# AwsGeek/thinvids

Hardware: AMD Instinct MI355X
Metric: encoded frames/sec (whole node) at fixed PSNR, 1080p & 4K HEVC, 1/2/4/8 MI355X (higher is better)
Workload: dtype uint8 video / int32 integer transforms (bit-exact HEVC)

## Files before the change

### csrc/core/capi.cpp

```cpp
#include <cstring>
#include <exception>
#include <memory>
#include <string>
#include <vector>

#include "tv/av1_enc.h"
#include "tv/container.h"
#include "tv/cpu_encoder.h"
#include "tv/hevc_codec.h"
#include "tv/me_model.h"
#include "tv/sdh.h"
#include "tv/synth.h"
#include "tv/synth_tile.h"
#include "tv/tb_frag.h"

using namespace tv;

namespace {
thread_local std::string g_err;
template <class F> int guard(F&& f) {
  try {
    f();
    return 0;
  } catch (const std::exception& e) {
    g_err = e.what();
    return -1;
  }
}
struct Bytes {
  std::vector<uint8_t> v;
};

struct TileOctave {
  int nx = 0;
  std::vector<uint8_t> lat;
  std::vector<uint16_t> top;
  std::vector<int> cy, sy;
  void build(int lp, uint32_t seed, const std::vector<int32_t>& px, const std::vector<int32_t>& py) {
    const SynthWin w = synth_win(lp, seed, px.front(), px.back(), py.front(), py.back());
    nx = (int)px.size();
    lat.resize((size_t)w.npx * w.npy);
    for (int r = 0; r < w.npy; ++r)
      for (int i = 0; i < w.npx; ++i) lat[(size_t)r * w.npx + i] = (uint8_t)synth_win_lattice(w, i, r);
    top.resize((size_t)w.npy * nx);
    for (int x = 0; x < nx; ++x) {
      int ci, sx;
      synth_axis(px[x], w.sh, w.cx0, ci, sx);
      for (int r = 0; r < w.npy; ++r)
        top[(size_t)r * nx + x] = (uint16_t)synth_top(lat[(size_t)r * w.npx + ci], lat[(size_t)r * w.npx + ci + 1], sx);
    }
    cy.resize(py.size());
    sy.resize(py.size());
    for (size_t y = 0; y < py.size(); ++y) synth_axis(py[y], w.sh, w.cy0, cy[y], sy[y]);
  }
  int at(int x, int y) const {
    const uint16_t* t = &top[(size_t)cy[y] * nx + x];
    return synth_rows(t[0], t[nx], sy[y]);
  }
};

void synth_tile_fill(const SynthFrameCtx& f, int c, int x0, int y0, int nx, int ny, int pw, uint8_t* P) {
  const int s = c ? 1 : 0, dw = c ? f.W / 2 : f.W, dh = c ? f.H / 2 : f.H;
  const bool tex = synth_textured(f.seed);
  std::vector<int32_t> px(nx), py(ny), qx(nx), qy(ny);
  for (int x = 0; x < nx; ++x) px[x] = synth_tile_pos(x0 + x, dw, s);
  for (int y = 0; y < ny; ++y) py[y] = synth_tile_pos(y0 + y, dh, s);
  std::vector<int> v((size_t)nx * ny);
  TileOctave oct[4];
  for (int x = 0; x < nx; ++x) qx[x] = px[x] + f.t * synth_pan_x(tex);
  for (int y = 0; y < ny; ++y) qy[y] = py[y] + f.t * synth_pan_y(tex);
  const int nb = synth_bg_octaves(c, tex);
  for (int i = 0; i < nb; ++i) oct[i].build(synth_bg_lp(c, i), synth_bg_seed(f.seed, c, i), qx, qy);
  for (int y = 0; y < ny; ++y)
    for (int x = 0; x < nx; ++x) {
      int n[4] = {0, 0, 0, 0};
      for (int i = 0; i < nb; ++i) n[i] = oct[i].at(x, y);
      v[(size_t)y * nx + x] = synth_bg_mix(c, tex, n);
    }
  for (int k = 0; k < kSynthObjects; ++k) {
    const SynthObject& o = f.obj[k];
    int32_t xlo, xhi, ylo, yhi;
    synth_obj_range(px.front(), px.back(), f.ox[k], o.w, xlo, xhi);
    synth_obj_range(py.front(), py.back(), f.oy[k], o.h, ylo, yhi);
    if (xlo > xhi || ylo > yhi) continue;
    for (int x = 0; x < nx; ++x) qx[x] = clip3(xlo, xhi, px[x] - f.ox[k]);
    for (int y = 0; y < ny; ++y) qy[y] = clip3(ylo, yhi, py[y] - f.oy[k]);
    const int no = synth_obj_octaves(c), base = synth_obj_base(f.seed, k, c);
    for (int i = 0; i < no; ++i) oct[i].build(synth_obj_lp(c, i), synth_obj_seed(o, c, i), qx, qy);
    for (int y = 0; y < ny; ++y)
      for (int x = 0; x < nx; ++x) {
        const int32_t rx16 = px[x] - f.ox[k], ry16 = py[y] - f.oy[k];
        if (rx16 != qx[x] || ry16 != qy[y] || synth_cover_col(o, rx16) > synth_cover_row(o, ry16)) continue;
        int n[2] = {0, 0};
        for (int i = 0; i < no; ++i) n[i] = oct[i].at(x, y);
        v[(size_t)y * nx + x] = synth_obj_mix(c, base, n);
      }
  }
  for (int y = 0; y < ny; ++y)
    for (int x = 0; x < nx; ++x) {
      int r = v[(size_t)y * nx + x];
      if (tex) r += synth_grain(f.seed, f.t, c, tv_min(x0 + x, dw - 1), tv_min(y0 + y, dh - 1));
      P[(size_t)(y0 + y) * pw + x0 + x] = (uint8_t)clip_pixel(r);
    }
}
}

extern "C" {

const char* tv_last_error() { return g_err.c_str(); }
int tv_core_version() { return 1; }

void* tv_bytes_new() { return new Bytes(); }
void tv_bytes_free(void* b) { delete static_cast<Bytes*>(b); }
size_t tv_bytes_size(void* b) { return static_cast<Bytes*>(b)->v.size(); }
const uint8_t* tv_bytes_data(void* b) { return static_cast<Bytes*>(b)->v.data(); }
void tv_bytes_clear(void* b) { static_cast<Bytes*>(b)->v.clear(); }

void tv_synth_frame(uint32_t seed, int t, int W, int H, uint8_t* y, uint8_t* u, uint8_t* v) {
  SynthFrameCtx ctx;
  synth_frame_ctx(seed, t, W, H, ctx);
  for (int c = 0; c < 3; ++c) {
    uint8_t* P = c == 0 ? y : (c == 1 ? u : v);
    const int w = c ? W / 2 : W, h = c ? H / 2 : H;
    for (int j = 0; j < h; ++j)
      for (int i = 0; i < w; ++i) P[(size_t)j * w + i] = (uint8_t)synth_sample_ctx(ctx, c, i, j);
  }
}

void tv_synth_frame_tiled(uint32_t seed, int t, int W, int H, int tile_w, int tile_h, uint8_t* y, uint8_t* u,
                          uint8_t* v) {
  SynthFrameCtx ctx;
  synth_frame_ctx(seed, t, W, H, ctx);
  const int cw = (W + kCtb - 1) / kCtb * kCtb, ch = (H + kCtb - 1) / kCtb * kCtb;
  for (int c = 0; c < 3; ++c) {
    uint8_t* P = c == 0 ? y : (c == 1 ? u : v);
    const int pw = c ? cw / 2 : cw, ph = c ? ch / 2 : ch;
    for (int y0 = 0; y0 < ph; y0 += tile_h)
      for (int x0 = 0; x0 < pw; x0 += tile_w)
        synth_tile_fill(ctx, c, x0, y0, tv_min(tile_w, pw - x0), tv_min(tile_h, ph - y0), pw, P);
  }
}

int tv_satd8x8(const int* d, int stride) { return satd8x8(d, stride); }

void* tv_cpu_encoder_new(int width, int height, int qp, int deblock, int range, int max_merge) {
  SeqConfig cfg;
  cfg.width = width;
  cfg.height = height;
  cfg.qp = qp;
  cfg.set_flags(deblock);
  cfg.max_merge_cand = max_merge;
  cfg.finalize();
  CpuEncoder* e = nullptr;
  guard([&] { e = new CpuEncoder(cfg, range); });
  return e;
}
void* tv_cpu_encoder_new_b(int width, int height, int qp, int deblock, int range, int max_merge, int mgop) {
  SeqConfig cfg;
  cfg.width = width;
  cfg.height = height;
  cfg.qp = qp;
  cfg.set_flags(deblock);
  cfg.max_merge_cand = max_merge;
  cfg.mgop = mgop;
  cfg.finalize();
  CpuEncoder* e = nullptr;
  guard([&] { e = new CpuEncoder(cfg, range); });
  return e;
}
int tv_cpu_encoder_begin_gop(void* e, int nframes, int* disp) {
  return guard([&] {
    auto* enc = static_cast<CpuEncoder*>(e);
    enc->begin_gop(nframes);
    for (size_t k = 0; k < enc->plan().pics.size(); ++k) disp[k] = enc->plan().pics[k].disp;
  });
}
int tv_gop_plan(int nframes, int mgop, int* disp, int* type, int* ref0, int* ref1, int* layer, int* info) {
  const GopPlan g = plan_gop(nframes, mgop);
  for (size_t k = 0; k < g.pics.size(); ++k) {
    disp[k] = g.pics[k].disp;
    type[k] = g.pics[k].type;
    ref0[k] = g.pics[k].ref[0];
    ref1[k] = g.pics[k].ref[1];
    layer[k] = g.pics[k].layer;
  }
  info[0] = g.dpb_size;
  info[1] = g.num_reorder;
  return (int)g.pics.size();
}
void* tv_cpu_encoder_new_crf(int width, int height, int qp, int deblock, int range, int max_merge, int crf) {
  SeqConfig cfg;
  cfg.width = width;
  cfg.height = height;
  cfg.qp = qp;
  cfg.set_flags(deblock);
  cfg.max_merge_cand = max_merge;
  cfg.crf = crf;
  cfg.finalize();
  CpuEncoder* e = nullptr;
  guard([&] { e = new CpuEncoder(cfg, range); });
  return e;
}
void tv_cpu_encoder_free(void* e) { delete static_cast<CpuEncoder*>(e); }
int tv_cpu_encoder_encode(void* e, const uint8_t* y, const uint8_t* u, const uint8_t* v, int sy,
                          int sc, int idr, int poc, void* out) {
  return guard([&] {
    const uint8_t* planes[3] = {y, u, v};
    const int strides[3] = {sy, sc, sc};
    static_cast<CpuEncoder*>(e)->encode_frame(planes, strides, idr != 0, poc, static_cast<Bytes*>(out)->v);
  });
}
int tv_cpu_encoder_encode_qp(void* e, const uint8_t* y, const uint8_t* u, const uint8_t* v, int sy, int sc, int idr,
                             int poc, int qp, void* out) {
  return guard([&] {
    const uint8_t* planes[3] = {y, u, v};
    const int strides[3] = {sy, sc, sc};
    static_cast<CpuEncoder*>(e)->encode_frame(planes, strides, idr != 0, poc, static_cast<Bytes*>(out)->v, qp);
  });
}
void tv_cpu_encoder_recon(void* e, uint8_t* y, uint8_t* u, uint8_t* v) {
  const Picture& p = static_cast<CpuEncoder*>(e)->recon();
  std::memcpy(y, p.y.data(), p.y.size());
  std::memcpy(u, p.u.data(), p.u.size());
  std::memcpy(v, p.v.data(), p.v.size());
}
void tv_cpu_encoder_decisions(void* e, uint8_t* cu_log2, uint8_t* intra, uint8_t* ipm, int16_t* mv,
                              uint8_t* cbf) {
  const FrameDecisions& d = static_cast<CpuEncoder*>(e)->dec;
  std::memcpy(cu_log2, d.cu_log2.data(), d.cu_log2.size());
  std::memcpy(intra, d.intra.data(), d.intra.size());
  std::memcpy(ipm, d.ipm.data(), d.ipm.size());
  std::memcpy(mv, d.mv.data(), d.mv.size() * 2);
  std::memcpy(cbf, d.cbf.data(), d.cbf.size());
}
void tv_cpu_encoder_levels(void* e, int16_t* cy, int16_t* cu, int16_t* cv) {
  const FrameDecisions& d = static_cast<CpuEncoder*>(e)->dec;
  std::memcpy(cy, d.coef_y.data(), d.coef_y.size() * 2);
  std::memcpy(cu, d.coef_u.data(), d.coef_u.size() * 2);
  std::memcpy(cv, d.coef_v.data(), d.coef_v.size() * 2);
}

int tv_reconstruct_frame(int width, int height, int qp, int deblock, const uint8_t* src_y,
                         const uint8_t* src_u, const uint8_t* src_v, const uint8_t* ref_y,
                         const uint8_t* ref_u, const uint8_t* ref_v, const uint8_t* cu_log2,
                         const uint8_t* intra, const uint8_t* ipm, const int16_t* mv,
                         uint8_t* cbf_out, int16_t* cy, int16_t* cu, int16_t* cv, uint8_t* rec_y,
                         uint8_t* rec_u, uint8_t* rec_v) {
  return guard([&] {
    SeqConfig cfg;
    cfg.width = width;
    cfg.height = height;
    cfg.qp = qp;
    cfg.deblock = (deblock & ~kFlagSignHiding) != 0;
    cfg.sign_hiding = (deblock & kFlagSignHiding) != 0;
    cfg.rqt = false;
    cfg.finalize();
    const int W = cfg.coded_w, H = cfg.coded_h;
    Picture src, ref, rec;
    src.alloc(W, H);
    rec.alloc(W, H);
    std::memcpy(src.y.data(), src_y, src.y.size());
    std::memcpy(src.u.data(), src_u, src.u.size());
    std::memcpy(src.v.data(), src_v, src.v.size());
    if (ref_y) {
      ref.alloc(W, H);
      std::memcpy(ref.y.data(), ref_y, ref.y.size());
      std::memcpy(ref.u.data(), ref_u, ref.u.size());
      std::memcpy(ref.v.data(), ref_v, ref.v.size());
    }
    FrameDecisions fd;
    fd.alloc(W, H);
    std::memcpy(fd.cu_log2.data(), cu_log2, fd.cu_log2.size());
    std::memcpy(fd.intra.data(), intra, fd.intra.size());
    std::memcpy(fd.ipm.data(), ipm, fd.ipm.size());
    std::memcpy(fd.mv.data(), mv, fd.mv.size() * 2);
    reconstruct_frame(cfg, src, ref_y ? &ref : nullptr, fd, rec);
    std::memcpy(cbf_out, fd.cbf.data(), fd.cbf.size());
    std::memcpy(cy, fd.coef_y.data(), fd.coef_y.size() * 2);
    std::memcpy(cu, fd.coef_u.data(), fd.coef_u.size() * 2);
    std::memcpy(cv, fd.coef_v.data(), fd.coef_v.size() * 2);
    std::memcpy(rec_y, rec.y.data(), rec.y.size());
    std::memcpy(rec_u, rec.u.data(), rec.u.size());
    std::memcpy(rec_v, rec.v.data(), rec.v.size());
  });
}

int tv_write_frame(int width, int height, int qp, int deblock, int max_merge, int idr, int poc,
                   const uint8_t* cu_log2, const uint8_t* intra, const uint8_t* ipm,
                   const int16_t* mv, const uint8_t* cbf, const int16_t* cy, const int16_t* cu,
                   const int16_t* cv, void* out) {
  return guard([&] {
    SeqConfig cfg;
    cfg.width = width;
    cfg.height = height;
    cfg.qp = qp;
    cfg.deblock = (deblock & ~kFlagSignHiding) != 0;
    cfg.sign_hiding = (deblock & kFlagSignHiding) != 0;
    cfg.max_merge_cand = max_merge;
    cfg.finalize();
    FrameData f;
    f.w8 = cfg.w8();
    f.h8 = cfg.h8();
    f.cu_log2 = cu_log2;
    f.intra = intra;
    f.ipm = ipm;
    f.mv = mv;
    f.cbf = cbf;
    f.coef[0] = cy;
    f.coef[1] = cu;
    f.coef[2] = cv;
    auto& o = static_cast<Bytes*>(out)->v;
    if (idr) write_parameter_sets(cfg, o);
    write_slice(cfg, f, poc, idr != 0, o);
  });
}

void* tv_decoder_new() { return new HevcDecoder(); }
void tv_decoder_free(void* d) { delete static_cast<HevcDecoder*>(d); }
int tv_decoder_decode(void* d, const uint8_t* data, size_t n) {
  return guard([&] { static_cast<HevcDecoder*>(d)->decode(data, n); });
}
int tv_decoder_decode_range(void* d, const uint8_t* data, size_t n, int first, int count) {
  return guard([&] { static_cast<HevcDecoder*>(d)->decode_range(data, n, first, count); });
}
void tv_hevc_scale_mv(int mvx, int mvy, int td, int tb, int* out) {
  const Mv m = scale_mv(Mv{mvx, mvy}, td, tb);
  out[0] = m.x;
  out[1] = m.y;
}
int tv_hevc_display_offsets(const uint8_t* data, size_t n, int* out, int cap) {
  int r = -1;
  guard([&] {
    const std::vector<int> off = display_offsets(data, n);
    for (int i = 0; i < (int)off.size() && i < cap; ++i) out[i] = off[i];
    r = (int)off.size();
  });
  return r;
}
int tv_hevc_probe(const uint8_t* data, size_t n, int* w, int* h, int* pictures, int* idrs) {
  return guard([&] {
    const StreamInfo s = probe_annexb(data, n);
    *w = s.width;
    *h = s.height;
    *pictures = s.pictures;
    *idrs = s.idrs;
  });
}
void tv_decoder_info(void* d, int* w, int* h, int* cw, int* ch, int* nframes) {
  auto* D = static_cast<HevcDecoder*>(d);
  *w = D->width;
  *h = D->height;
  *cw = D->coded_w;
  *ch = D->coded_h;
  *nframes = (int)D->pictures.size();
}
int tv_decoder_frame(void* d, int idx, int cropped, uint8_t* y, uint8_t* u, uint8_t* v) {
  return guard([&] {
    auto* D = static_cast<HevcDecoder*>(d);
    const Picture& p = D->pictures.at(idx).pic;
    const int w = cropped ? D->width : p.w, h = cropped ? D->height : p.h;
    for (int c = 0; c < 3; ++c) {
      uint8_t* dst = c == 0 ? y : (c == 1 ? u : v);
      const int cw = c ? w / 2 : w, chh = c ? h / 2 : h, sw = p.pw(c);
      for (int j = 0; j < chh; ++j) std::memcpy(dst + (size_t)j * cw, p.plane(c) + (size_t)j * sw, cw);
    }
  });
}

int tv_mux_mp4(const uint8_t* annexb, size_t n, int w, int h, int fps_num, int fps_den, void* out) {
  return guard([&] { static_cast<Bytes*>(out)->v = mux_mp4(annexb, n, w, h, fps_num, fps_den); });
}
int tv_mux_mp4_file(const uint8_t* const* segs, const size_t* sizes, int nseg, int w, int h, int fps_num, int fps_den,
                    const char* path, unsigned long long* out_size) {
  return guard([&] { *out_size = mux_mp4_file(segs, sizes, nseg, w, h, fps_num, fps_den, path); });
}
int tv_mux_file(const uint8_t* const* segs, const size_t* sizes, int nseg, int w, int h, int fps_num, int fps_den,
                const SideTrack* tracks, int ntracks, int container, const char* path, unsigned long long* out_size) {
  return guard([&] {
    *out_size = mux_file(segs, sizes, nseg, w, h, fps_num, fps_den, tracks, ntracks, container, path);
  });
}
size_t tv_side_track_size() { return sizeof(SideTrack); }

void tv_mv_rate(const int* dx, const int* dy, int n, int* est, int* idx) {
  for (int i = 0; i < n; ++i) {
    est[i] = mv_bits_est(dx[i], dy[i]);
    idx[i] = me_pen_index(dx[i], dy[i]);
  }
}
void tv_av1_mv_comp_bits(const int* d, int n, int* bits) {
  for (int i = 0; i < n; ++i) bits[i] = av1::mv_comp_bits(d[i]);
}
int tv_tb_frag_expand(int which, int* out) {
  static constexpr TbFragTables t = make_tb_frag();
  if (which < 0 || which >= 8) return 0;
  const int side = which < 2 ? 32 : 16;
  for (int n = 0; n < side; ++n)
    for (int k = 0; k < side; ++k)
      out[n * side + k] = int_of_f16_bits(which < 2 ? t.t32[which][n][k] : t.c16[(which - 2) >> 1][which & 1][n][k]);
  return side;
}
void tv_quant_levels(const int* coef, int n, int qp, int log2N, int* ref, int* fast) {
  const QuantParams q = quant_params(qp, log2N);
  for (int i = 0; i < n; ++i) {
    ref[i] = quant_level(coef[i], qp, log2N, false);
    fast[i] = quant_fast(coef[i], q);
  }
}
void tv_sdh_deltas(const int* coef, int n, int qp, int log2N, int intra, int* ref, int* fast) {
  const QuantParams q = quant_params(qp, log2N);
  for (int i = 0; i < n; ++i) {
    const int l = quant_level(coef[i], qp, log2N, intra != 0);
    ref[i] = sdh_delta(coef[i], l, qp, log2N);
    fast[i] = sdh_delta_fast(coef[i], l, q);
  }
}
int tv_demux_mp4(const uint8_t* mp4, size_t n, int* w, int* h, int* nframes, int* timescale,
                 int* delta, void* out) {
  return guard([&] { static_cast<Bytes*>(out)->v = demux_mp4(mp4, n, w, h, nframes, timescale, delta); });
}

}
```

### csrc/gpu/k_frame.hip

```cpp
#include <cstring>

#include "gpu_common.h"
#include "k_encode.h"
#include "tv/synth.h"
#include "tv/synth_tile.h"

namespace tv {
namespace gpu {

constexpr int kSynTW = kSynthTileW, kSynTH = kSynthTileH, kSynRows = kSynTH / 4;
static_assert(kSynTW == 256 && kSynTH % 4 == 0, "a wave of 4-sample items spans the tile; 4 waves share its rows");

struct SynthArgs {
  SynthObject obj[kSynthObjects];
  int32_t t[kMaxBatch];
  int32_t ox[kMaxBatch][kSynthObjects], oy[kMaxBatch][kSynthObjects];
};
static_assert(sizeof(SynthArgs) + sizeof(Geo) + sizeof(FrameSet) + 16 <= 4096, "kernel arguments are limited to 4 KB");

constexpr int kSynSpanX = (kSynTW - 1) * 16, kSynSpanY = (kSynTH - 1) * 16;
constexpr int syn_max(int a, int b) { return a > b ? a : b; }
constexpr int syn_pts(int lp, int s) { return synth_win_max(kSynSpanX << s, lp) * synth_win_max(kSynSpanY << s, lp); }
constexpr int syn_rows(int lp, int s) { return synth_win_max(kSynSpanY << s, lp); }
constexpr int syn_lat_size(bool tex) {
  return syn_max(syn_max(syn_pts(7, 0) + syn_pts(5, 0) + syn_pts(3, 0) + (tex ? syn_pts(1, 0) : 0), syn_pts(4, 0) + syn_pts(2, 0)),
                 syn_max(syn_pts(8, 1), syn_pts(5, 1)));
}
constexpr int syn_top_rows(bool tex) {
  return syn_max(syn_max(syn_rows(7, 0) + syn_rows(5, 0) + syn_rows(3, 0) + (tex ? syn_rows(1, 0) : 0), syn_rows(4, 0) + syn_rows(2, 0)),
                 syn_max(syn_rows(8, 1), syn_rows(5, 1)));
}

__device__ __forceinline__ void syn_lattice(const SynthWin& w, uint8_t* lat, int wave, int lane) {
  for (int r = wave; r < w.npy; r += 4)
    for (int i = lane; i < w.npx; i += 64) lat[r * w.npx + i] = (uint8_t)synth_win_lattice(w, i, r);
}
__device__ __forceinline__ void syn_top(const SynthWin& w, const uint8_t* lat, uint16_t* top, int col, int32_t p16) {
  int ci, sx;
  synth_axis(p16, w.sh, w.cx0, ci, sx);
  for (int r = 0; r < w.npy; ++r)
    top[r * kSynTW + col] = (uint16_t)synth_top(lat[r * w.npx + ci], lat[r * w.npx + ci + 1], sx);
}
__device__ __forceinline__ void syn_eval(const SynthWin& w, const uint16_t* top, int x, int32_t p16, int n[4]) {
  int cy, sy;
  synth_axis(p16, w.sh, w.cy0, cy, sy);
  const uint2 a = *reinterpret_cast<const uint2*>(top + cy * kSynTW + x);
  const uint2 b = *reinterpret_cast<const uint2*>(top + (cy + 1) * kSynTW + x);
  n[0] = synth_rows((int)(a.x & 0xffff), (int)(b.x & 0xffff), sy);
  n[1] = synth_rows((int)(a.x >> 16), (int)(b.x >> 16), sy);
  n[2] = synth_rows((int)(a.y & 0xffff), (int)(b.y & 0xffff), sy);
  n[3] = synth_rows((int)(a.y >> 16), (int)(b.y >> 16), sy);
}

template <bool kTex, bool kChroma>
__device__ __forceinline__ void syn_tile(uint16_t* top, uint8_t* lat, FrameSet src, const Geo& g, uint32_t seed,
                                         const SynthArgs& a, int c, int x0, int y0) {
  constexpr int kBg = kChroma ? 1 : (kTex ? 4 : 3), kOb = kChroma ? 1 : 2, s = kChroma ? 1 : 0;
  __builtin_assume(kChroma ? c != 0 : c == 0);
  const int b = blockIdx.y;
  const int pw = g.W >> s, ph = g.H >> s, dw = g.dw >> s, dh = g.dh >> s;
  const int t = a.t[b];
  const int tid = threadIdx.x, lane = tid & 63, wave = __builtin_amdgcn_readfirstlane(tid >> 6);
  const int32_t tx0 = synth_tile_pos(x0, dw, s), tx1 = synth_tile_pos(x0 + kSynTW - 1, dw, s);
  const int32_t ty0 = synth_tile_pos(y0, dh, s), ty1 = synth_tile_pos(y0 + kSynTH - 1, dh, s);
  const int32_t colp = synth_tile_pos(x0 + tid, dw, s);
  const int x = 4 * lane, yw = y0 + wave * kSynRows;
  int32_t sp[4];
#pragma unroll
  for (int j = 0; j < 4; ++j) sp[j] = synth_tile_pos(x0 + x + j, dw, s);

  SynthWin w[kBg];
  int lat0[kBg], row0[kBg];
  const int panx = t * synth_pan_x(kTex), pany = t * synth_pan_y(kTex);
  {
    int lo = 0, ro = 0;
#pragma unroll
    for (int i = 0; i < kBg; ++i) {
      w[i] = synth_win(synth_bg_lp(c, i), synth_bg_seed(seed, c, i), tx0 + panx, tx1 + panx, ty0 + pany, ty1 + pany);
      lat0[i] = lo;
      row0[i] = ro;
      syn_lattice(w[i], lat + lo, wave, lane);
      lo += w[i].npx * w[i].npy;
      ro += w[i].npy;
    }
  }
  __syncthreads();
#pragma unroll
  for (int i = 0; i < kBg; ++i) syn_top(w[i], lat + lat0[i], top + row0[i] * kSynTW, tid, colp + panx);
  __syncthreads();
  uint32_t word[kSynRows];
#pragma unroll
  for (int j = 0; j < kSynRows; ++j) {
    const int32_t py = synth_tile_pos(yw + j, dh, s) + pany;
    int n[4][4] = {};
#pragma unroll
    for (int i = 0; i < kBg; ++i) syn_eval(w[i], top + row0[i] * kSynTW, x, py, n[i]);
    word[j] = 0;
#pragma unroll
    for (int q = 0; q < 4; ++q) {
      const int m[4] = {n[0][q], n[1][q], n[2][q], n[3][q]};
      word[j] |= (uint32_t)synth_bg_mix(c, kTex, m) << (8 * q);
    }
  }

  for (int k = 0; k < kSynthObjects; ++k) {
    const SynthObject& o = a.obj[k];
    const int32_t ox = a.ox[b][k], oy = a.oy[b][k];
    int32_t xlo, xhi, ylo, yhi;
    synth_obj_range(tx0, tx1, ox, o.w, xlo, xhi);
    synth_obj_range(ty0, ty1, oy, o.h, ylo, yhi);
    if (xlo > xhi || ylo > yhi) continue;
    const int base = synth_obj_base(seed, k, c);
    SynthWin wo[kOb];
    int olat[kOb], orow[kOb];
    __syncthreads();
    {
      int lo = 0, ro = 0;
#pragma unroll
      for (int i = 0; i < kOb; ++i) {
        wo[i] = synth_win(synth_obj_lp(c, i), synth_obj_seed(o, c, i), xlo, xhi, ylo, yhi);
        olat[i] = lo;
        orow[i] = ro;
        syn_lattice(wo[i], lat + lo, wave, lane);
        lo += wo[i].npx * wo[i].npy;
        ro += wo[i].npy;
      }
    }
    __syncthreads();
#pragma unroll
    for (int i = 0; i < kOb; ++i) syn_top(wo[i], lat + olat[i], top + orow[i] * kSynTW, tid, clip3(xlo, xhi, colp - ox));
    __syncthreads();
    int64_t cover[4];
#pragma unroll
    for (int q = 0; q < 4; ++q) {
      const int32_t rx16 = sp[q] - ox;
      cover[q] = rx16 < xlo || rx16 > xhi ? INT64_MAX : synth_cover_col(o, rx16);
    }
#pragma unroll
    for (int j = 0; j < kSynRows; ++j) {
      const int32_t ry16 = synth_tile_pos(yw + j, dh, s) - oy;
      if (ry16 < ylo || ry16 > yhi) continue;
      const int64_t cover_row = synth_cover_row(o, ry16);
      int n[2][4] = {};
#pragma unroll
      for (int i = 0; i < kOb; ++i) syn_eval(wo[i], top + orow[i] * kSynTW, x, ry16, n[i]);
#pragma unroll
      for (int q = 0; q < 4; ++q) {
        if (cover[q] > cover_row) continue;
        const int m[2] = {n[0][q], n[1][q]};
        word[j] = (word[j] & ~(0xffu << (8 * q))) | (uint32_t)synth_obj_mix(c, base, m) << (8 * q);
      }
    }
  }

  if (x0 + x >= pw) return;
  uint8_t* P = src.plane(c, b, g);
#pragma unroll
  for (int j = 0; j < kSynRows; ++j) {
    const int y = yw + j;
    if (y >= ph) break;
    uint32_t out = word[j];
    if (kTex) {
      const int yc = tv_min(y, dh - 1);
      out = 0;
#pragma unroll
      for (int q = 0; q < 4; ++q) {
        const int v = (int)((word[j] >> (8 * q)) & 255) + synth_grain(seed, t, c, tv_min(x0 + x + q, dw - 1), yc);
        out |= (uint32_t)clip_pixel(v) << (8 * q);
      }
    }
    *reinterpret_cast<uint32_t*>(P + (long)y * pw + x0 + x) = out;
  }
}

template <bool kTex>
__global__ void __launch_bounds__(256) k_synth(FrameSet src, Geo g, uint32_t seed, SynthArgs a) {
  __shared__ __attribute__((aligned(8))) uint16_t top[syn_top_rows(kTex) * kSynTW];
  __shared__ uint8_t lat[syn_lat_size(kTex)];
  const int nlx = (g.W + kSynTW - 1) / kSynTW, ncx = (g.W / 2 + kSynTW - 1) / kSynTW;
  const int nl = nlx * ((g.H + kSynTH - 1) / kSynTH), nc = ncx * ((g.H / 2 + kSynTH - 1) / kSynTH);
  int id = blockIdx.x, c = 0;
  if (id >= nl) {
    c = id >= nl + nc ? 2 : 1;
    id -= nl + (c - 1) * nc;
  }
  const int ntx = c ? ncx : nlx, ty = id / ntx, x0 = (id - ty * ntx) * kSynTW, y0 = ty * kSynTH;
  if (c)
    syn_tile<kTex, true>(top, lat, src, g, seed, a, c, x0, y0);
  else
    syn_tile<kTex, false>(top, lat, src, g, seed, a, 0, x0, y0);
}

__global__ void __launch_bounds__(256) k_sse(FrameSet a, FrameSet r, Geo g, unsigned long long* sse) {
  const int c = blockIdx.y, b = blockIdx.z;
  const int pw = c ? g.W / 2 : g.W;
  const int dw = c ? g.dw / 2 : g.dw, dh = c ? g.dh / 2 : g.dh;
  const uint8_t* A = a.plane(c, b, g);
  const uint8_t* R = r.plane(c, b, g);
  const int wq = (dw + 3) >> 2;
  unsigned s = 0;
  for (int i = blockIdx.x * blockDim.x + threadIdx.x; i < wq * dh; i += gridDim.x * blockDim.x) {
    const int y = i / wq, x = (i - y * wq) * 4;
    const uint32_t va = *reinterpret_cast<const uint32_t*>(A + (long)y * pw + x);
    const uint32_t vr = *reinterpret_cast<const uint32_t*>(R + (long)y * pw + x);
#pragma unroll
    for (int k = 0; k < 4; ++k) {
      const int d = (int)((va >> (8 * k)) & 255) - (int)((vr >> (8 * k)) & 255);
      s += (x + k < dw) ? (unsigned)(d * d) : 0u;
    }
  }
  unsigned long long t = s;
  for (int o = 32; o > 0; o >>= 1) t += __shfl_xor(t, o, 64);
  __shared__ unsigned long long part[4];
  if ((threadIdx.x & 63) == 0) part[threadIdx.x >> 6] = t;
  __syncthreads();
  if (threadIdx.x == 0) atomicAdd(sse + b * 3 + c, part[0] + part[1] + part[2] + part[3]);
}

typedef short tv_short2 __attribute__((ext_vector_type(2)));

__device__ constexpr uint32_t pack_taps4(int f, int k0) {
  return (uint32_t)(uint8_t)kLumaFilter[f][k0] | (uint32_t)(uint8_t)kLumaFilter[f][k0 + 1] << 8 |
         (uint32_t)(uint8_t)kLumaFilter[f][k0 + 2] << 16 | (uint32_t)(uint8_t)kLumaFilter[f][k0 + 3] << 24;
}
__device__ constexpr uint32_t pack_taps2(int f, int k0) {
  return (uint32_t)(uint16_t)kLumaFilter[f][k0] | (uint32_t)(uint16_t)kLumaFilter[f][k0 + 1] << 16;
}
__device__ __forceinline__ int dot4(uint32_t a, uint32_t b, int c) {
  return __builtin_amdgcn_sdot4((int)a, (int)b, c, false);
}
__device__ __forceinline__ int dot2(uint32_t a, uint32_t b, int c) {
  return __builtin_amdgcn_sdot2(__builtin_bit_cast(tv_short2, a), __builtin_bit_cast(tv_short2, b), c, false);
}
__device__ __forceinline__ uint32_t pack4_pixels(int v0, int v1, int v2, int v3) {
  return (uint32_t)clip_pixel(v0) | (uint32_t)clip_pixel(v1) << 8 | (uint32_t)clip_pixel(v2) << 16 |
         (uint32_t)clip_pixel(v3) << 24;
}

constexpr int kPhW = 10;
__global__ void __launch_bounds__(256) k_phase_planes(FrameSet ref, uint8_t* phase, Geo g) {
  const int tid = threadIdx.x;
  const int L = xcd_remap(blockIdx.x + gridDim.x * (blockIdx.y + gridDim.y * blockIdx.z),
                          gridDim.x * gridDim.y * gridDim.z);
  const int tpf = gridDim.x * gridDim.y, b = L / tpf, tyi = (L - b * tpf) / gridDim.x;
  const int tx0 = (L - b * tpf - tyi * gridDim.x) * 32 - 8, ty0 = tyi * 32 - 8;
  const uint8_t* R = ref.plane(0, b, g);
  __shared__ uint32_t raw[39][kPhW];
  __shared__ __align__(16) int16_t hf[3][39][32];
  for (int i = tid; i < 39 * kPhW; i += 256) {
    const int rr = i / kPhW, w = i - rr * kPhW;
    const uint8_t* row = R + (long)clip3(0, g.H - 1, ty0 - 3 + rr) * g.W;
    const int x = tx0 - 4 + 4 * w;
    uint32_t v;
    if (x >= 0 && x + 3 < g.W) {
      v = *reinterpret_cast<const uint32_t*>(row + x);
    } else {
      v = 0;
#pragma unroll
      for (int k = 0; k < 4; ++k) v |= (uint32_t)row[clip3(0, g.W - 1, x + k)] << (8 * k);
    }
    raw[rr][w] = v ^ 0x80808080u;
  }
  __syncthreads();
  for (int i = tid; i < 39 * 8; i += 256) {
    const int rr = i >> 3, c4 = i & 7;
    const uint32_t w0 = raw[rr][c4], w1 = raw[rr][c4 + 1], w2 = raw[rr][c4 + 2];
    int out[3][4];
#pragma unroll
    for (int j = 0; j < 4; ++j) {
      const uint32_t lo = j == 3 ? w1 : __builtin_amdgcn_alignbyte(w1, w0, j + 1);
      const uint32_t hi = j == 3 ? w2 : __builtin_amdgcn_alignbyte(w2, w1, j + 1);
#pragma unroll
      for (int f = 1; f < 4; ++f) out[f - 1][j] = dot4(lo, pack_taps4(f, 0), dot4(hi, pack_taps4(f, 4), 8192));
    }
#pragma unroll
    for (int f = 0; f < 3; ++f) {
      uint2 v;
      v.x = (uint32_t)(uint16_t)out[f][0] | (uint32_t)out[f][1] << 16;
      v.y = (uint32_t)(uint16_t)out[f][2] | (uint32_t)out[f][3] << 16;
      *reinterpret_cast<uint2*>(&hf[f][rr][4 * c4]) = v;
    }
  }
  __syncthreads();
  const int r = tid >> 3, c0 = (tid & 7) * 4;
  const int X = tx0 + c0, Y = ty0 + r;
  if (X + 8 >= g.pw16 || Y >= g.H + 8) return;
  uint8_t* base = phase + (long)b * 16 * g.psz + (long)(Y + 8) * g.pw16 + (X + 8);
  auto store = [&](int plane, uint32_t w) { *reinterpret_cast<uint32_t*>(base + (long)plane * g.psz) = w; };
  {
    uint32_t R8[8];
#pragma unroll
    for (int k = 0; k < 8; ++k) R8[k] = raw[r + k][(c0 >> 2) + 1];
    store(0, R8[3] ^ 0x80808080u);
    uint32_t C[2][4];
#pragma unroll
    for (int h = 0; h < 2; ++h) {
      const uint32_t* q = R8 + 4 * h;
      const uint32_t t01l = __builtin_amdgcn_perm(q[1], q[0], 0x05010400u);
      const uint32_t t01h = __builtin_amdgcn_perm(q[1], q[0], 0x07030602u);
      const uint32_t t23l = __builtin_amdgcn_perm(q[3], q[2], 0x05010400u);
      const uint32_t t23h = __builtin_amdgcn_perm(q[3], q[2], 0x07030602u);
      C[h][0] = __builtin_amdgcn_perm(t23l, t01l, 0x05040100u);
      C[h][1] = __builtin_amdgcn_perm(t23l, t01l, 0x07060302u);
      C[h][2] = __builtin_amdgcn_perm(t23h, t01h, 0x05040100u);
      C[h][3] = __builtin_amdgcn_perm(t23h, t01h, 0x07060302u);
    }
#pragma unroll
    for (int fy = 1; fy < 4; ++fy) {
      int v[4];
#pragma unroll
      for (int j = 0; j < 4; ++j)
        v[j] = dot4(C[0][j], pack_taps4(fy, 0), dot4(C[1][j], pack_taps4(fy, 4), 8192 + 32)) >> 6;
      store(4 * fy, pack4_pixels(v[0], v[1], v[2], v[3]));
    }
  }
#pragma unroll
  for (int fx = 1; fx < 4; ++fx) {
    uint2 H8[8];
#pragma unroll
    for (int k = 0; k < 8; ++k) H8[k] = *reinterpret_cast<const uint2*>(&hf[fx - 1][r + k][c0]);
    {
      const int h0 = (int16_t)(H8[3].x & 0xffff), h1 = (int16_t)(H8[3].x >> 16);
      const int h2 = (int16_t)(H8[3].y & 0xffff), h3 = (int16_t)(H8[3].y >> 16);
      store(fx, pack4_pixels((h0 + 32) >> 6, (h1 + 32) >> 6, (h2 + 32) >> 6, (h3 + 32) >> 6));
    }
    uint32_t P[4][4];
#pragma unroll
    for (int m = 0; m < 4; ++m) {
      P[m][0] = __builtin_amdgcn_perm(H8[2 * m + 1].x, H8[2 * m].x, 0x05040100u);
      P[m][1] = __builtin_amdgcn_perm(H8[2 * m + 1].x, H8[2 * m].x, 0x07060302u);
      P[m][2] = __builtin_amdgcn_perm(H8[2 * m + 1].y, H8[2 * m].y, 0x05040100u);
      P[m][3] = __builtin_amdgcn_perm(H8[2 * m + 1].y, H8[2 * m].y, 0x07060302u);
    }
#pragma unroll
    for (int fy = 1; fy < 4; ++fy) {
      int v[4];
#pragma unroll
      for (int j = 0; j < 4; ++j) {
        int a = dot2(P[0][j], pack_taps2(fy, 0), 0);
        a = dot2(P[1][j], pack_taps2(fy, 2), a);
        a = dot2(P[2][j], pack_taps2(fy, 4), a);
        a = dot2(P[3][j], pack_taps2(fy, 6), a);
        v[j] = ((a >> 6) + 32) >> 6;
      }
      store(fx + 4 * fy, pack4_pixels(v[0], v[1], v[2], v[3]));
    }
  }
}

__global__ void __launch_bounds__(256) __attribute__((amdgpu_waves_per_eu(8, 8))) k_deblock(FrameSet rec, DecisionSet dec, Geo g, int horizontal) {
  const int b = blockIdx.y;
  const int qp = dec.qp[b];
  const long ub = b * g.usz;
  const uint8_t* cl = dec.cu_log2 + ub;
  const uint8_t* in = dec.intra + ub;
  const uint8_t* cb = dec.cbf + ub;
  const int16_t* mv = dec.mv + 2 * ub;
  const uint8_t* dir = dec.dir ? dec.dir + ub : nullptr;
  const int16_t* mv1 = dec.mv1 ? dec.mv1 + 2 * ub : nullptr;
  const uint8_t* tu = dec.tu ? dec.tu + ub : nullptr;
  uint8_t* Y = rec.plane(0, b, g);
  uint8_t* U = rec.plane(1, b, g);
  uint8_t* V = rec.plane(2, b, g);
  const int W = g.W, H = g.H, Wc = W / 2;
  const int qpc = chroma_qp(qp, 0);
  const int nl = horizontal ? (H / 8 - 1) * (W / 4) : (W / 8 - 1) * (H / 4);
  const int nc = horizontal ? (H / 16 - 1) * (Wc / 4) : (W / 16 - 1) * (H / 8);
  auto ld = [](const uint8_t* p) { return *reinterpret_cast<const uint32_t*>(p); };
  auto st = [](uint8_t* p, uint32_t v) { *reinterpret_cast<uint32_t*>(p) = v; };
  for (int i = blockIdx.x * blockDim.x + threadIdx.x; i < nl + nc; i += gridDim.x * blockDim.x) {
    if (i < nl) {
      if (!horizontal) {
        const int x = 8 * (1 + i % (W / 8 - 1)), y = 4 * (i / (W / 8 - 1));
        const int bs = deblock_edge_bs(cl, in, cb, mv, g.w8, x - 1, y, x, y, dir, mv1, tu);
        if (bs) {
          uint32_t v[4][2];
#pragma unroll
          for (int k = 0; k < 4; ++k) {
            v[k][0] = ld(Y + (long)(y + k) * W + x - 4);
            v[k][1] = ld(Y + (long)(y + k) * W + x);
          }
          deblock_luma_edge4(reinterpret_cast<uint8_t*>(&v[0][1]), 1, 8, bs, qp);
#pragma unroll
          for (int k = 0; k < 4; ++k) {
            st(Y + (long)(y + k) * W + x - 4, v[k][0]);
            st(Y + (long)(y + k) * W + x, v[k][1]);
          }
        }
      } else {
        const int y = 8 * (1 + i % (H / 8 - 1)), x = 4 * (i / (H / 8 - 1));
        const int bs = deblock_edge_bs(cl, in, cb, mv, g.w8, x, y - 1, x, y, dir, mv1, tu);
        if (bs) {
          uint32_t v[8];
#pragma unroll
          for (int r = 0; r < 8; ++r) v[r] = ld(Y + (long)(y - 4 + r) * W + x);
          deblock_luma_edge4(reinterpret_cast<uint8_t*>(&v[4]), 4, 1, bs, qp);
#pragma unroll
          for (int r = 1; r < 7; ++r) st(Y + (long)(y - 4 + r) * W + x, v[r]);
        }
      }
    } else {
      const int j = i - nl;
      if (!horizontal) {
        const int xc = 8 * (1 + j % (W / 16 - 1)), yc = 4 * (j / (W / 16 - 1));
        const int bs = deblock_edge_bs(cl, in, cb, mv, g.w8, 2 * xc - 1, 2 * yc, 2 * xc, 2 * yc, dir, mv1, tu);
        if (bs == 2) {
#pragma unroll
          for (int pl = 0; pl < 2; ++pl) {
            uint8_t* P = pl ? V : U;
            uint32_t v[4][2];
#pragma unroll
            for (int k = 0; k < 4; ++k) {
              v[k][0] = ld(P + (long)(yc + k) * Wc + xc - 4);
              v[k][1] = ld(P + (long)(yc + k) * Wc + xc);
            }
            deblock_chroma_edge(reinterpret_cast<uint8_t*>(&v[0][1]), 1, 8, 4, qpc);
#pragma unroll
            for (int k = 0; k < 4; ++k) {
              st(P + (long)(yc + k) * Wc + xc - 4, v[k][0]);
              st(P + (long)(yc + k) * Wc + xc, v[k][1]);
            }
          }
        }
      } else {
        const int yc = 8 * (1 + j % (H / 16 - 1)), xc = 4 * (j / (H / 16 - 1));
        const int bs = deblock_edge_bs(cl, in, cb, mv, g.w8, 2 * xc, 2 * yc - 1, 2 * xc, 2 * yc, dir, mv1, tu);
        if (bs == 2) {
#pragma unroll
          for (int pl = 0; pl < 2; ++pl) {
            uint8_t* P = pl ? V : U;
            uint32_t v[4];
#pragma unroll
            for (int r = 0; r < 4; ++r) v[r] = ld(P + (long)(yc - 2 + r) * Wc + xc);
            deblock_chroma_edge(reinterpret_cast<uint8_t*>(&v[2]), 4, 1, 4, qpc);
            st(P + (long)(yc - 1) * Wc + xc, v[1]);
            st(P + (long)yc * Wc + xc, v[2]);
          }
        }
      }
    }
  }
}

void launch_synth(FrameSet src, const Geo& g, uint32_t seed, const FrameIdx& fi, int B, hipStream_t s) {
  SynthArgs a;
  std::memset(&a, 0, sizeof a);
  SynthFrameCtx f;
  for (int b = 0; b < B; ++b) {
    synth_frame_ctx(seed, fi.t[b], g.dw, g.dh, f);
    a.t[b] = f.t;
    std::memcpy(a.ox[b], f.ox, sizeof f.ox);
    std::memcpy(a.oy[b], f.oy, sizeof f.oy);
  }
  if (B > 0) std::memcpy(a.obj, f.obj, sizeof f.obj);
  auto tiles = [](int w, int h) { return ((w + kSynTW - 1) / kSynTW) * ((h + kSynTH - 1) / kSynTH); };
  dim3 grid((unsigned)(tiles(g.W, g.H) + 2 * tiles(g.W / 2, g.H / 2)), (unsigned)B);
  if (synth_textured(seed))
    k_synth<true><<<grid, 256, 0, s>>>(src, g, seed, a);
  else
    k_synth<false><<<grid, 256, 0, s>>>(src, g, seed, a);
}
__global__ void __launch_bounds__(256) k_gather_frames(const uint8_t* frames, long seg_stride, FrameSet src, Geo g,
                                                       int B) {
  const long f16 = (g.ysz + 2 * g.csz) / 16, y16 = g.ysz / 16, c16 = g.csz / 16;
  for (long i = (long)blockIdx.x * 256 + threadIdx.x; i < B * f16; i += (long)gridDim.x * 256) {
    const int b = (int)(i / f16);
    const long r = i - b * f16;
    const uint4 v = reinterpret_cast<const uint4*>(frames + b * seg_stride)[r];
    uint4* d = r < y16 ? reinterpret_cast<uint4*>(src.y + b * g.ysz) + r
               : r < y16 + c16 ? reinterpret_cast<uint4*>(src.u + b * g.csz) + (r - y16)
                               : reinterpret_cast<uint4*>(src.v + b * g.csz) + (r - y16 - c16);
    *d = v;
  }
}
void launch_gather_frames(const uint8_t* frames, long seg_stride, FrameSet src, const Geo& g, int B, hipStream_t s) {
  const long n = B * (g.ysz + 2 * g.csz) / 16;
  k_gather_frames<<<(unsigned)tv_min(4096L, (n + 255) / 256), 256, 0, s>>>(frames, seg_stride, src, g, B);
}
struct QpArgs {
  int8_t q[64];
};
__global__ void __launch_bounds__(64) k_set_qp(int8_t* dst, QpArgs a, int n) {
  if ((int)threadIdx.x < n) dst[threadIdx.x] = a.q[threadIdx.x];
}
void launch_set_qp(int8_t* dst, const int8_t* host, int n, hipStream_t s) {
  for (int o = 0; o < n; o += 64) {
    QpArgs a;
    const int m = n - o < 64 ? n - o : 64;
    std::memcpy(a.q, host + o, (size_t)m);
    k_set_qp<<<1, 64, 0, s>>>(dst + o, a, m);
  }
}

void launch_sse(FrameSet a, FrameSet r, const Geo& g, unsigned long long* sse, int B, hipStream_t s) {
  dim3 grid((unsigned)tv_min(256, (int)((g.ysz / 4 + 4095) / 4096)), 3, B);
  k_sse<<<grid, 256, 0, s>>>(a, r, g, sse);
}
void launch_phase_planes(FrameSet ref, uint8_t* phase, const Geo& g, int B, hipStream_t s) {
  dim3 grid((g.W + 16 + 31) / 32, (g.H + 16 + 31) / 32, B);
  k_phase_planes<<<grid, 256, 0, s>>>(ref, phase, g);
}
constexpr int kSaoT = 34;
constexpr int kSaoTc = 18;
constexpr int kSaoP = kSaoT + 2, kSaoPc = kSaoTc + 2;
constexpr int kSaoTile = kSaoT * kSaoP + 2 * kSaoTc * kSaoPc;
constexpr int kSaoStage = (kSaoTile + 255) / 256;
__device__ __forceinline__ int sao_tix(int c, int row, int col) {
  return c == 0 ? row * kSaoP + col + 1 : kSaoT * kSaoP + (c - 1) * kSaoTc * kSaoPc + row * kSaoPc + col + 1;
}
typedef short sao_s2 __attribute__((ext_vector_type(2)));
__device__ __forceinline__ sao_s2 sao_pair(uint32_t w) { return __builtin_bit_cast(sao_s2, w); }
typedef unsigned short sao_u2 __attribute__((ext_vector_type(2)));
__device__ __forceinline__ sao_s2 sao_sign2(sao_s2 d) {
  const sao_s2 z = {0, 0};
  const sao_u2 f = {15, 15};
  return (d >> 15) | __builtin_bit_cast(sao_s2, __builtin_bit_cast(sao_u2, z - d) >> f);
}
__device__ __forceinline__ sao_s2 sao_relu2(sao_s2 e) { return e & ~(e >> 15); }
__device__ __forceinline__ sao_s2 sao_pkmax(sao_s2 a, sao_s2 b) {
  uint32_t r;
  asm("v_pk_max_i16 %0, %1, %2" : "=v"(r) : "v"(__builtin_bit_cast(uint32_t, a)), "v"(__builtin_bit_cast(uint32_t, b)));
  return sao_pair(r);
}
__device__ __forceinline__ sao_s2 sao_pkmin(sao_s2 a, sao_s2 b) {
  uint32_t r;
  asm("v_pk_min_i16 %0, %1, %2" : "=v"(r) : "v"(__builtin_bit_cast(uint32_t, a)), "v"(__builtin_bit_cast(uint32_t, b)));
  return sao_pair(r);
}

__device__ __forceinline__ void sao_tile_pos(int i, int& c, int& j) {
  c = i < kSaoT * kSaoT ? 0 : (i < kSaoT * kSaoT + kSaoTc * kSaoTc ? 1 : 2);
  j = c == 0 ? i : i - kSaoT * kSaoT - (c - 1) * kSaoTc * kSaoTc;
}

__global__ void __launch_bounds__(256) k_sao_decide(FrameSet src, FrameSet deb, FrameSet out, uint32_t* sao, Geo g,
                                                    const int8_t* qp, const RcTables* rc,
                                                    unsigned long long* sse) {
  const int tid = threadIdx.x, lane = tid & 63;
  int ctu, b;
  xcd_ctb(ctu, b);
  const long long lam16 = rc->sao_lam16[qp[b]];
  const int cx = ctu % g.wc, cy = ctu / g.wc;
  __shared__ SaoStats st[3];
  __shared__ __align__(16) int16_t tile[kSaoTile];
  __shared__ int bpos[3];
  __shared__ int bh[3][32][16];
  for (int i = tid; i < 3 * (int)(sizeof(SaoStats) / 4); i += 256) reinterpret_cast<int*>(st)[i] = 0;
  if (kSaoBandOffsets)
    for (int i = tid; i < 3 * 32 * 16; i += 256) (&bh[0][0][0])[i] = 0;
  {
    uint32_t* tile32 = reinterpret_cast<uint32_t*>(tile);
    uint32_t v[3];
    int at[3], dw[3], nd[3];
    bool act[3], in[3];
#pragma unroll
    for (int k = 0; k < 3; ++k) {
      int c, row, d;
      if (k < 2) {
        const int i = tid + 256 * k;
        c = 0;
        row = i / 10;
        d = i - 10 * row;
        act[k] = i < 34 * 10;
      } else {
        const int pl = tid >= 108 ? 1 : 0, j = tid - 108 * pl;
        c = 1 + pl;
        row = j / 6;
        d = j - 6 * row;
        act[k] = tid < 2 * 108;
      }
      const int n = c ? 16 : 32, w = c ? g.W / 2 : g.W, h = c ? g.H / 2 : g.H;
      const int x = cx * n - 4 + 4 * d, y = cy * n - 1 + row;
      in[k] = act[k] && x >= 0 && x < w && y >= 0 && y < h;
      v[k] = in[k] ? *reinterpret_cast<const uint32_t*>(deb.plane(c, b, g) + (long)y * w + x) : 0u;
      at[k] = (sao_tix(c, row, -1) >> 1) + 2 * d - 1;
      dw[k] = d;
      nd[k] = c ? 6 : 10;
    }
#pragma unroll
    for (int k = 0; k < 3; ++k) {
      if (!act[k]) continue;
      const uint32_t lo = in[k] ? __builtin_amdgcn_perm(0u, v[k], 0x0c010c00u) : 0xFFFFFFFFu;
      const uint32_t hi = in[k] ? __builtin_amdgcn_perm(0u, v[k], 0x0c030c02u) : 0xFFFFFFFFu;
      if (dw[k] >= 1) tile32[at[k]] = lo;
      if (dw[k] < nd[k] - 1) tile32[at[k] + 1] = hi;
    }
  }
  const int wave = __builtin_amdgcn_readfirstlane(tid >> 6);
  const int c = wave < 2 ? 0 : wave - 1;
  const int n = c ? 16 : 32, w = c ? g.W / 2 : g.W;
  const int nsh = c ? 4 : 5;
  const int iters = c ? 4 : 8;
  const uint8_t* S = src.plane(c, b, g) + (long)(cy * n) * w + cx * n;
  static_assert(!kSaoBandOffsets, "the packed statistics carry no band histogram");
  const bool interior = cx > 0 && cy > 0 && cx < g.wc - 1 && cy < g.hc - 1;
  const int piters = c ? 2 : 4;
  int sv[8] = {};
  uint32_t sp[4] = {};
  if (interior) {
#pragma unroll
    for (int k = 0; k < 4; ++k) {
      const int pidx = lane + 64 * k;
      const int ly = (c == 0 ? wave * 16 : 0) + (pidx >> (nsh - 1)), lx = 2 * (pidx & ((n >> 1) - 1));
      sp[k] = k < piters ? *reinterpret_cast<const uint16_t*>(S + ly * w + lx) : 0u;
    }
  } else {
#pragma unroll
    for (int k = 0; k < 8; ++k) {
      const int i = (c == 0 ? wave * 512 : 0) + lane + 64 * k;
      sv[k] = k < iters ? S[(i >> nsh) * w + (i & (n - 1))] : 0;
    }
  }
  __syncthreads();
  int eo[4][4];
  if (interior) {
    const uint32_t* tile32 = reinterpret_cast<const uint32_t*>(tile);
    sao_s2 acc[4][4];
#pragma unroll
    for (int d = 0; d < 4; ++d)
#pragma unroll
      for (int q = 0; q < 4; ++q) acc[d][q] = sao_s2{0, 0};
    const sao_s2 zero = {0, 0}, one = {1, 1}, mone = {-1, -1}, sixteen = {16, 16};
#pragma unroll
    for (int k = 0; k < 4; ++k) {
      if (k >= piters) break;
      const int pidx = lane + 64 * k;
      const int ly = (c == 0 ? wave * 16 : 0) + (pidx >> (nsh - 1)), lx = 2 * (pidx & ((n >> 1) - 1));
      uint32_t Pv[3], Cv[3], Nv[3];
#pragma unroll
      for (int r = 0; r < 3; ++r) {
        const int i0 = sao_tix(c, ly + r, lx + 1) >> 1;
        Pv[r] = tile32[i0 - 1];
        Cv[r] = tile32[i0];
        Nv[r] = tile32[i0 + 1];
      }
      sao_s2 L[3], R[3], Cc[3];
#pragma unroll
      for (int r = 0; r < 3; ++r) {
        L[r] = sao_pair(__builtin_amdgcn_alignbyte(Cv[r], Pv[r], 2));
        R[r] = sao_pair(__builtin_amdgcn_alignbyte(Nv[r], Cv[r], 2));
        Cc[r] = sao_pair(Cv[r]);
      }
      const sao_s2 v = Cc[1];
      const uint32_t o = sp[k];
      const sao_s2 orig = {(short)(o & 255), (short)(o >> 8)};
      const sao_s2 w = (orig - v) * sixteen + one;
      const sao_s2 A[4] = {L[1], Cc[0], L[0], R[0]}, Bn[4] = {R[1], Cc[2], R[2], L[2]};
#pragma unroll
      for (int d = 0; d < 4; ++d) {
        const sao_s2 e = sao_pkmin(sao_pkmax(v - A[d], mone), one) + sao_pkmin(sao_pkmax(v - Bn[d], mone), one);
        const sao_s2 pos = sao_pkmax(e, zero), neg = sao_pkmax(zero - e, zero);
        const sao_s2 is[4] = {neg >> one, neg & one, pos & one, pos >> one};
#pragma unroll
        for (int q = 0; q < 4; ++q) acc[d][q] += w * is[q];
      }
    }
#pragma unroll
    for (int d = 0; d < 4; ++d)
#pragma unroll
      for (int q = 0; q < 4; ++q) {
        const int F = __builtin_amdgcn_sdot2(acc[d][q], one, 0, false), C = F & 15;
        eo[d][q] = (F - C) * 128 + C;
      }
  } else {
    unsigned long long eo64[4] = {0, 0, 0, 0};
#pragma unroll
    for (int k = 0; k < 8; ++k) {
      if (k >= iters) break;
      const int i = (c == 0 ? wave * 512 : 0) + lane + 64 * k;
      const int lx = i & (n - 1), ly = i >> nsh;
      const int v = tile[sao_tix(c, ly + 1, lx + 1)];
      const int d16 = (sv[k] - v) * 16 + 1;
      const unsigned long long p64 = (unsigned long long)(long long)d16;
#pragma unroll
      for (int d = 0; d < 4; ++d) {
        int dx, dy;
        sao_eo_dir(d, dx, dy);
        const int a = tile[sao_tix(c, ly + 1 + dy, lx + 1 + dx)], bb = tile[sao_tix(c, ly + 1 - dy, lx + 1 - dx)];
        const int e = tv_min(tv_max(v - a, -1), 1) + tv_min(tv_max(v - bb, -1), 1);
        const int f = e + 2 - (e > 0);
        eo64[d] += (a >= 0 && bb >= 0 && e != 0) ? p64 << (16 * f) : 0ull;
      }
      if (kSaoBandOffsets) atomicAdd(&bh[c][v >> 3][lane & 15], (sv[k] - v) * 2048 + 1);
    }
#pragma unroll
    for (int d = 0; d < 4; ++d) {
      unsigned long long acc = eo64[d];
#pragma unroll
      for (int q = 0; q < 4; ++q) {
        const int fv = (int)(int16_t)(acc & 0xffffu);
        acc = (acc - (unsigned long long)(long long)fv) >> 16;
        const int cnt = fv & 15;
        eo[d][q] = ((fv - cnt) >> 4) * 2048 + cnt;
      }
    }
  }
  {
    int t[16];
#pragma unroll
    for (int k = 0; k < 16; ++k) t[k] = eo[k >> 2][k & 3];
#pragma unroll
    for (int j = 0; j < 8; ++j) {
      const auto r = __builtin_amdgcn_permlane32_swap((unsigned)t[j], (unsigned)t[j + 8], false, false);
      t[j] = (int)(r[0] + r[1]);
    }
#pragma unroll
    for (int j = 0; j < 4; ++j) {
      const auto r = __builtin_amdgcn_permlane16_swap((unsigned)t[j], (unsigned)t[j + 4], false, false);
      t[j] = (int)(r[0] + r[1]);
    }
    const int m8 = -((lane >> 3) & 1), m4 = -((lane >> 2) & 1);
#pragma unroll
    for (int j = 0; j < 2; ++j) {
      const int x = (t[j] ^ t[j + 2]) & m8;
      t[j] = (t[j] ^ x) + dpp::mov<dpp::kRowRor8>(t[j + 2] ^ x);
    }
    {
      const int x = (t[0] ^ t[1]) & m4;
      t[0] = (t[0] ^ x) + __shfl_xor(t[1] ^ x, 4, 64);
    }
    int tot = t[0];
    tot += dpp::mov<dpp::kQuadXor1>(tot);
    tot += dpp::mov<dpp::kQuadXor2>(tot);
    const int k = lane >> 2;
    if ((lane & 3) == 0 && (tot & 2047)) {
      atomicAdd(&st[c].eo_n[k >> 2][(k & 3) + 1], tot & 2047);
      atomicAdd(&st[c].eo_s[k >> 2][(k & 3) + 1], (tot - (tot & 2047)) / 2048);
    }
  }
  __shared__ SaoTables tab;
  __shared__ uint32_t prm[3];
  __syncthreads();
  if (kSaoBandOffsets && tid < 96) {
    const int cc = tid >> 5, band = tid & 31;
    int tot = 0;
#pragma unroll
    for (int k = 0; k < 16; ++k) tot += bh[cc][band][k];
    st[cc].bo_n[band] = tot & 2047;
    st[cc].bo_s[band] = (tot - (tot & 2047)) / 2048;
  }
  __syncthreads();
  if (tid < kSaoItems && (kSaoBandOffsets || tid % 48 < 16)) sao_item(st, lam16, tid, tab);
  __syncthreads();
  if (kSaoBandOffsets && tid < 96) sao_window(tid, tab);
  __syncthreads();
  if (!kSaoBandOffsets) {
    if (tid < 3) bpos[tid] = 0;
  } else if (wave < 3) {
    long long j = lane < 32 ? tab.win_j[wave][lane] : LLONG_MAX;
    int p = lane < 32 ? lane : 64;
#pragma unroll
    for (int o = 32; o >= 1; o >>= 1) {
      const long long j2 = __shfl_xor(j, o);
      const int p2 = __shfl_xor(p, o);
      if (j2 < j || (j2 == j && p2 < p)) {
        j = j2;
        p = p2;
      }
    }
    if (lane == 0) bpos[wave] = p;
  }
  __syncthreads();
  if (tid == 0) {
    sao_finish_pos(tab, lam16, bpos, prm);
    uint32_t* o = sao + 3 * ((long)b * g.wc * g.hc + ctu);
    o[0] = prm[0];
    o[1] = prm[1];
    o[2] = prm[2];
  }
  __syncthreads();
  static_assert(!kSaoBandOffsets, "the SAO filter has no band-offset path");
  unsigned e2[3] = {0, 0, 0};
  const uint32_t* tile32 = reinterpret_cast<const uint32_t*>(tile);
  for (int i = tid; i < 256 + 128; i += 256) {
    const int cc = i < 256 ? 0 : (i < 320 ? 1 : 2);
    const int j = cc == 0 ? i : i - 256 - (cc - 1) * 64;
    const int nd = cc ? 4 : 8, nn = cc ? 16 : 32, ww = cc ? g.W / 2 : g.W;
    const int ly = j >> (cc ? 2 : 3), lx0 = 4 * (j & (nd - 1));
    const uint32_t p = prm[cc];
    const long at = (long)(cy * nn + ly) * ww + cx * nn + lx0;
    const int dwc = cc ? g.dw / 2 : g.dw, dhc = cc ? g.dh / 2 : g.dh;
    const bool want_sse = sse && cy * nn + ly < dhc;
    const uint32_t sw = want_sse ? *reinterpret_cast<const uint32_t*>(src.plane(cc, b, g) + at) : 0u;
    uint32_t word = 0;
    const int i0 = sao_tix(cc, ly + 1, lx0 + 1) >> 1;
    const uint32_t C0 = tile32[i0], C1 = tile32[i0 + 1];
    if (sao_type(p) == 2) {
      int dx, dy;
      sao_eo_dir(sao_class(p), dx, dy);
      const int pd = (cc ? kSaoPc : kSaoP) >> 1;
      const int ra = i0 + dy * pd, rb = i0 - dy * pd;
      const uint32_t Wa[4] = {tile32[ra - 1], tile32[ra], tile32[ra + 1], tile32[ra + 2]};
      const uint32_t Wb[4] = {tile32[rb - 1], tile32[rb], tile32[rb + 1], tile32[rb + 2]};
      auto shifted = [](const uint32_t* W, int k, int s) -> uint32_t {
        return s == 0 ? W[k + 1] : s < 0 ? __builtin_amdgcn_alignbyte(W[k + 1], W[k], 2)
                                         : __builtin_amdgcn_alignbyte(W[k + 2], W[k + 1], 2);
      };
      const uint32_t t0 = ((p >> 7) & 15) | ((p >> 11) & 15) << 8 | 8u << 16 | ((p >> 15) & 15) << 24;
      const uint32_t t1 = (p >> 19) & 15;
      const sao_s2 two = {2, 2}, eight = {8, 8};
      const sao_u2 u8s = {8, 8};
      uint32_t r2[2];
#pragma unroll
      for (int k = 0; k < 2; ++k) {
        const sao_s2 v = sao_pair(k ? C1 : C0);
        const sao_s2 A = sao_pair(shifted(Wa, k, dx)), B = sao_pair(shifted(Wb, k, -dx));
        const sao_s2 inv = (A | B) >> 15;
        const sao_s2 e = (sao_sign2(v - A) + sao_sign2(v - B)) & ~inv;
        const uint32_t sel = __builtin_bit_cast(uint32_t, e + two) | 0x0c000c00u;
        const sao_s2 off = sao_pair(__builtin_amdgcn_perm(t1, t0, sel));
        const sao_s2 r = sao_relu2(v + off - eight);
        r2[k] = __builtin_bit_cast(uint32_t, r | (sao_s2{0, 0} - __builtin_bit_cast(sao_s2, __builtin_bit_cast(sao_u2, r) >> u8s)));
      }
      word = __builtin_amdgcn_perm(r2[1], r2[0], 0x06040200u);
    } else {
      word = __builtin_amdgcn_perm(C1, C0, 0x06040200u);
    }
    *reinterpret_cast<uint32_t*>(out.plane(cc, b, g) + at) = word;
    if (want_sse) {
      if (cx * nn + lx0 + 4 <= dwc) {
#pragma unroll
        for (int h = 0; h < 2; ++h) {
          const uint32_t sel = h ? 0x0c030c02u : 0x0c010c00u;
          const sao_s2 d = sao_pair(__builtin_amdgcn_perm(0u, sw, sel)) - sao_pair(__builtin_amdgcn_perm(0u, word, sel));
          const sao_u2 dd = __builtin_bit_cast(sao_u2, d * d);
          e2[cc] = __builtin_amdgcn_udot2(dd, sao_u2{1, 1}, e2[cc], false);
        }
      } else {
#pragma unroll
        for (int q = 0; q < 4; ++q) {
          const int d = (int)((sw >> (8 * q)) & 255) - (int)((word >> (8 * q)) & 255);
          e2[cc] += cx * nn + lx0 + q < dwc ? (unsigned)(d * d) : 0u;
        }
      }
    }
  }
  if (sse) {
    __shared__ unsigned long long esum[3];
    if (tid < 3) esum[tid] = 0;
    __syncthreads();
#pragma unroll
    for (int c2 = 0; c2 < 3; ++c2) {
      const int t = wave_sum((int)e2[c2]);
      if (lane == 0 && t) atomicAdd(&esum[c2], (unsigned long long)(unsigned)t);
    }
    __syncthreads();
    if (tid < 3 && esum[tid]) atomicAdd(sse + b * 3 + tid, esum[tid]);
  }
}

void launch_sao(FrameSet src, FrameSet deb, FrameSet out, uint32_t* sao, const int8_t* qp, const RcTables* rc,
                const Geo& g, int B, hipStream_t s, unsigned long long* sse) {
  k_sao_decide<<<dim3(g.wc * g.hc, B), 256, 0, s>>>(src, deb, out, sao, g, qp, rc, sse);
}

void launch_deblock(FrameSet rec, DecisionSet dec, const Geo& g, int B, hipStream_t s) {
  dim3 grid((unsigned)tv_min(1024, (int)(g.ysz / 32 / 256 + 1)), B);
  k_deblock<<<grid, 256, 0, s>>>(rec, dec, g, 0);
  k_deblock<<<grid, 256, 0, s>>>(rec, dec, g, 1);
}

}
}
```

### csrc/gpu/k_stage.hip

```cpp
#include <hip/hip_runtime.h>

#include <string>

#include "gpu_common.h"
#include "k_encode.h"

namespace tv {
namespace gpu {

__global__ void __launch_bounds__(256) k_pad_plane(const uint8_t* __restrict__ src, int sw, int sh, int sstride, long sfs,
                                                   uint8_t* __restrict__ dst, int pw, int ph, int dstride, long dfs) {
  const int f = blockIdx.z, y = blockIdx.y;
  const int x0 = (blockIdx.x * 256 + threadIdx.x) * 4;
  if (x0 >= pw) return;
  const uint8_t* S = src + f * sfs + (long)tv_min(y, sh - 1) * sstride;
  uint8_t* D = dst + f * dfs + (long)y * dstride;
#pragma unroll
  for (int k = 0; k < 4; ++k)
    if (x0 + k < pw) D[x0 + k] = S[tv_min(x0 + k, sw - 1)];
}

template <typename T>
__global__ void __launch_bounds__(256) k_thumbs8(const T* __restrict__ y, int tw, int stride, long fs, float* out,
                                                 float scale) {
  const int x = blockIdx.x * 256 + threadIdx.x, r = blockIdx.y, f = blockIdx.z;
  if (x >= tw) return;
  const T* p = y + (long)f * fs + (long)(8 * r) * stride + 8 * x;
  unsigned s = 0;
#pragma unroll
  for (int j = 0; j < 8; ++j)
#pragma unroll
    for (int i = 0; i < 8; ++i) s += p[(long)j * stride + i];
  out[((long)f * gridDim.y + r) * tw + x] = (float)s * scale / 64.0f;
}
}
}

namespace {
thread_local std::string g_stage_err;
int stage_status() {
  const hipError_t e = hipGetLastError();
  if (e == hipSuccess) return 0;
  g_stage_err = hipGetErrorString(e);
  return -1;
}
}

extern "C" {
const char* tv_stage_last_error() { return g_stage_err.c_str(); }

int tv_thumbs8_batch(const void* y, int bits, int w, int h, int stride, long fs, int n, float* out, void* stream) {
  const int tw = w / 8, th = h / 8;
  if (tw <= 0 || th <= 0 || th > 65535 || n <= 0 || n > 65535 || stride < w) {
    g_stage_err = "tv_thumbs8_batch: bad geometry";
    return -1;
  }
  const dim3 grid((unsigned)((tw + 255) / 256), (unsigned)th, (unsigned)n);
  hipStream_t st = static_cast<hipStream_t>(stream);
  if (bits > 8)
    tv::gpu::k_thumbs8<uint16_t><<<grid, 256, 0, st>>>(static_cast<const uint16_t*>(y), tw, stride, fs, out, 0.25f);
  else
    tv::gpu::k_thumbs8<uint8_t><<<grid, 256, 0, st>>>(static_cast<const uint8_t*>(y), tw, stride, fs, out, 1.0f);
  return stage_status();
}

int tv_pad_batch(const uint8_t* src, int sw, int sh, int sstride, long sfs, uint8_t* dst, int pw, int ph, int dstride,
                 long dfs, int n, void* stream) {
  if (sw <= 0 || sh <= 0 || pw < sw || ph < sh || dstride < pw || sstride < sw || n <= 0 || n > 65535 ||
      ph > 65535) {
    g_stage_err = "tv_pad_batch: bad geometry";
    return -1;
  }
  const dim3 grid((unsigned)((pw / 4 + 255) / 256 + 1), (unsigned)ph, (unsigned)n);
  tv::gpu::k_pad_plane<<<grid, 256, 0, static_cast<hipStream_t>(stream)>>>(src, sw, sh, sstride, sfs, dst, pw, ph,
                                                                          dstride, dfs);
  return stage_status();
}

int tv_synth_batch(uint8_t* dst, int w, int h, int n, const int* t, uint32_t seed, void* stream) {
  if (w < 2 || h < 2 || (w & 1) || (h & 1) || n <= 0) {
    g_stage_err = "tv_synth_batch: bad geometry";
    return -1;
  }
  const tv::gpu::Geo g = tv::gpu::make_geo(w, h);
  for (int b0 = 0; b0 < n; b0 += tv::gpu::kMaxBatch) {
    const int B = tv::tv_min(tv::gpu::kMaxBatch, n - b0);
    tv::gpu::FrameSet fs{dst + b0 * g.ysz, dst + n * g.ysz + b0 * g.csz, dst + n * g.ysz + n * g.csz + b0 * g.csz};
    tv::gpu::FrameIdx fi{};
    for (int b = 0; b < B; ++b) fi.t[b] = t[b0 + b];
    tv::gpu::launch_synth(fs, g, seed, fi, B, static_cast<hipStream_t>(stream));
  }
  return stage_status();
}
}
```

### thinvids_amd/_abi.py

```python
import ctypes as C

i, l, ll, sz, ull, f32 = C.c_int, C.c_long, C.c_longlong, C.c_size_t, C.c_ulonglong, C.c_float
i32, i64, u32, vp, cstr = C.c_int32, C.c_int64, C.c_uint32, C.c_void_p, C.c_char_p
u8p, i8p, i16p, i32p, u32p = (C.POINTER(t) for t in (C.c_uint8, C.c_int8, C.c_int16, C.c_int32, C.c_uint32))
i64p, u64p, lp, llp, ullp, szp = (C.POINTER(t) for t in (C.c_int64, C.c_uint64, l, ll, ull, sz))
f64p, vpp = C.POINTER(C.c_double), C.POINTER(vp)


class SideTrack(C.Structure):
    _fields_ = [("kind", i32), ("codec", i32), ("timescale", i32), ("channels", i32), ("sample_rate", i32),
                ("bits", i32), ("is_default", i32), ("reserved", i32), ("lang", C.c_char * 4), ("mkv_codec_id", cstr),
                ("priv", vp), ("priv_size", C.c_uint64), ("path", cstr), ("data", vp), ("nsamples", i64),
                ("offsets", vp), ("sizes", vp), ("pts", vp), ("durs", vp)]


CORE = {
    "tv_core_build_hash": (cstr, []),
    "tv_last_error": (cstr, []),
    "tv_core_version": (i, []),
    "tv_bytes_new": (vp, []),
    "tv_bytes_free": (None, [vp]),
    "tv_bytes_size": (sz, [vp]),
    "tv_bytes_data": (vp, [vp]),
    "tv_bytes_clear": (None, [vp]),
    "tv_synth_frame": (None, [u32, i, i, i, u8p, u8p, u8p]),
    "tv_synth_frame_tiled": (None, [u32, i, i, i, i, i, u8p, u8p, u8p]),
    "tv_satd8x8": (i, [i32p, i]),
    "tv_cpu_encoder_new": (vp, [i] * 6),
    "tv_cpu_encoder_new_b": (vp, [i] * 7),
    "tv_cpu_encoder_new_crf": (vp, [i] * 7),
    "tv_cpu_encoder_free": (None, [vp]),
    "tv_cpu_encoder_begin_gop": (i, [vp, i, i32p]),
    "tv_gop_plan": (i, [i, i] + [i32p] * 6),
    "tv_cpu_encoder_encode": (i, [vp, u8p, u8p, u8p, i, i, i, i, vp]),
    "tv_cpu_encoder_encode_qp": (i, [vp, u8p, u8p, u8p, i, i, i, i, i, vp]),
    "tv_cpu_encoder_recon": (None, [vp, u8p, u8p, u8p]),
    "tv_cpu_encoder_decisions": (None, [vp, u8p, u8p, u8p, i16p, u8p]),
    "tv_cpu_encoder_levels": (None, [vp, i16p, i16p, i16p]),
    "tv_reconstruct_frame": (i, [i] * 4 + [u8p] * 9 + [i16p, u8p, i16p, i16p, i16p, u8p, u8p, u8p]),
    "tv_write_frame": (i, [i] * 7 + [u8p, u8p, u8p, i16p, u8p, i16p, i16p, i16p, vp]),
    "tv_mv_rate": (None, [i32p, i32p, i, i32p, i32p]),
    "tv_av1_mv_comp_bits": (None, [i32p, i, i32p]),
    "tv_tb_frag_expand": (i, [i, i32p]),
    "tv_quant_levels": (None, [i32p, i, i, i, i32p, i32p]),
    "tv_sdh_deltas": (None, [i32p, i, i, i, i, i32p, i32p]),
    "tv_hevc_spec_table": (i, [cstr, i32p, i]),
    "tv_decoder_new": (vp, []),
    "tv_decoder_free": (None, [vp]),
    "tv_decoder_decode": (i, [vp, u8p, sz]),
    "tv_decoder_decode_range": (i, [vp, u8p, sz, i, i]),
    "tv_decoder_info": (None, [vp] + [i32p] * 5),
    "tv_decoder_frame": (i, [vp, i, i, u8p, u8p, u8p]),
    "tv_hevc_scale_mv": (None, [i, i, i, i, i32p]),
    "tv_hevc_display_offsets": (i, [u8p, sz, i32p, i]),
    "tv_hevc_probe": (i, [u8p, sz] + [i32p] * 4),
    "tv_mux_mp4": (i, [u8p, sz, i, i, i, i, vp]),
    "tv_mux_mp4_file": (i, [vpp, szp, i, i, i, i, i, cstr, ullp]),
    "tv_mux_file": (i, [vpp, szp, i, i, i, i, i, C.POINTER(SideTrack), i, i, cstr, ullp]),
    "tv_side_track_size": (sz, []),
    "tv_demux_mp4": (i, [u8p, sz] + [i32p] * 5 + [vp]),
    "tv_mp4s_open": (vp, [cstr, i, i, i, i, ull]),
    "tv_mp4s_append": (i, [vp, u8p, sz]),
    "tv_mp4s_close": (i, [vp, ullp]),
    "tv_mp4s_abort": (None, [vp]),
    "tv_mp4s_last_error": (cstr, []),
    "tv_io_last_error": (cstr, []),
    "tv_pread_parallel": (ll, [cstr, ll, ll, vp, i]),
    "tv_readahead": (i, [cstr, ll, ll]),
    "tv_av1c_last_error": (cstr, []),
    "tv_av1c_qlookup": (i, [i, i]),
    "tv_av1c_model_constants": (i, [i64p]),
    "tv_av1c_model_q": (None, [i, i64p]),
    "tv_av1c_golden_encode": (i, [i, i, i, u8p, i, i32p, i, vp, i64p, u8p, u32p, u32p, i16p, i16p, i16p, i32p, i8p,
                                  i32p, u8p]),
    "tv_av1c_ib_accept": (i, [u8p, i, i, u8p]),
    "tv_av1c_cfl_decide": (i, [u8p, u8p, u8p, i, i, i, i, i32p]),
    "tv_av1c_decode": (i, [u8p, sz, i, u8p, i32p, i32p]),
    "tv_av1c_probe": (i, [u8p, sz, i32p, i32p]),
    "tv_av1c_state_new": (vp, []),
    "tv_av1c_state_free": (None, [vp]),
    "tv_av1c_write_tu": (i, [vp, i, i, i32p, u32p, u32p, i16p, i16p, i16p, i8p, i32p, i, i, vp]),
    "tv_av1_last_error": (cstr, []),
    "tv_av1_cdef_find_dirs": (None, [u8p, i, i, u8p, i32p]),
    "tv_av1_cdef_search": (None, [u8p, u8p, i, i, i, u8p, i32p, i, i, u64p]),
    "tv_av1_cdef_apply": (None, [u8p, i, i, i, u8p, i32p, i, i, i8p, u8p]),
    "tv_av1_wiener_apply": (None, [u8p, i, i, i32p, u8p]),
    "tv_av1_wiener_stats": (None, [u8p, u8p, i, i, i, i32p, i64p]),
    "tv_av1_sgr_apply": (None, [u8p, i, i, i32p, u8p]),
    "tv_av1_sgr_stats": (None, [u8p, u8p, i, i, i, i64p]),
    "tv_av1_sgr_filter_planes": (None, [u8p, i, i, i, i32p, i32p]),
    "tv_av1_deblock": (i, [u8p, i, i, i, u32p, i, u8p]),
    "tv_av1_rc_roundtrip": (i, [i32p, i32p, i32p, i, i, i, vp, i32p]),
    "tv_av1_txfm_ref": (i, [i16p, i16p, i, i, i, i, i]),
    "tv_av1_txfm_basis": (i, [i, i, i32p]),
    "tv_mpeg2_last_error": (cstr, []),
    "tv_mpeg2_encode": (i, [i32p, i, i, u8p, vp, i64p, i32p, u8p]),
    "tv_mpeg2_probe": (i, [u8p, sz, i32p]),
    "tv_mpeg2_raps": (i, [u8p, sz, i64p, i64p, i32p, i32p, i]),
    "tv_mpeg2_decode": (i, [u8p, sz, i64, i64, i32, i32, i32, u8p, i32p, i64p]),
    "tv_mpeg2_table": (i, [i, i32p, i32p, i32p, i]),
    "tv_mpeg2_stat_name": (cstr, [i]),
    "tv_mpeg2_num_stats": (i, []),
}

GPU = {
    "tv_gpu_build_hash": (cstr, []),
    "tv_gpu_last_error": (cstr, []),
    "tv_gpu_device_count": (i, []),
    "tv_engine_new_b": (vp, [i] * 7 + [u32, i, i, i, i, i]),
    "tv_engine_free": (None, [vp]),
    "tv_engine_encode_synth": (i, [vp, i32p, i, i, vp]),
    "tv_engine_encode_host": (i, [vp, u8p, i, i, vp]),
    "tv_engine_encode_device": (i, [vp, vp, i, i, vp]),
    "tv_engine_segment_size": (sz, [vp, i]),
    "tv_engine_segment_copy": (None, [vp, i, u8p]),
    "tv_engine_sse": (None, [vp, i, f64p]),
    "tv_engine_timing": (None, [vp] + [f64p] * 4),
    "tv_engine_entropy_stats": (None, [vp, i32p, llp, i32p]),
    "tv_engine_entropy_host_pictures": (ll, [vp]),
    "tv_engine_entropy_lane_pictures": (ll, [vp, i]),
    "tv_engine_estimate": (i, [i] * 6 + [ullp, ullp]),
    "tv_engine_footprint": (None, [vp, ullp, ullp]),
    "tv_engine_last_recon": (i, [vp, i, u8p, u8p, u8p]),
    "tv_ingest_last_error": (cstr, []),
    "tv_ingest_h2d": (i, [cstr, ll, ll, vp, vp, ll, i, vp, f64p]),
    "tv_stage_last_error": (cstr, []),
    "tv_thumbs8_batch": (i, [vp, i, i, i, i, l, i, vp, vp]),
    "tv_pad_batch": (i, [vp, i, i, i, l, vp, i, i, i, l, i, vp]),
    "tv_synth_batch": (i, [vp, i, i, i, i32p, u32, vp]),
    "tv_ops_last_error": (cstr, []),
    "tv_resize_plane": (i, [vp, i, i, i, vp, i, i, i, vp, vp, i, vp, vp, i, vp, vp]),
    "tv_resize_batch": (i, [vp, i, i, i, l, vp, i, i, i, l, i, i, i, vp, vp, i, vp, vp, i, vp, i, i, i, vp]),
    "tv_rgb_to_i420": (i, [vp, i, i, i, vp, vp, vp, i, vp]),
    "tv_p010_to_i420": (i, [vp, vp, i, i, vp, vp, vp, vp]),
    "tv_tonemap_pq": (i, [vp, vp, i, i, vp, vp, vp, f32, f32, vp]),
    "tv_tonemap_pq_batch": (i, [vp, vp, i, i, i, vp, f32, f32, vp]),
    "tv_synth_p010": (i, [vp, vp, i, i, i, i, u32, vp]),
    "tv_overlay_mask": (i, [vp, i, i, i, vp, i, i, i, i, vp]),
    "tv_bwdif_segment": (i, [vp, vp, l, i, i, lp, i32p, i32p, i, vp]),
    "tv_bwdif_plane": (i, [vp, vp, vp, vp, i, i, i, vp]),
    "tv_ssim_plane": (i, [vp, vp, i, i, i, i, vp, vp]),
    "tv_av1_gpu_last_error": (cstr, []),
    "tv_gpu_cdef_dirs": (i, [vp, i, i, i, vp, vp, vp]),
    "tv_gpu_cdef_search": (i, [vp, vp, i, i, i, i, vp, vp, i, i, i, vp, vp, ull, i]),
    "tv_gpu_cdef_apply": (i, [vp, i, i, i, i, vp, vp, i, i, i, vp, vp, vp]),
    "tv_gpu_sgr_select": (i, [vp, vp, vp, i, i, i, i, vp, vp, vp, vp]),
    "tv_gpu_wiener_apply": (i, [vp, i, i, i, vp, vp, vp]),
    "tv_gpu_wiener_stats": (i, [vp, vp, i, i, i, i, vp, vp, vp]),
    "tv_gpu_sgr_stats": (i, [vp, vp, i, i, i, i, vp, vp]),
    "tv_gpu_sgr_apply": (i, [vp, i, i, i, vp, vp, vp]),
    "tv_gpu_av1_deblock_step": (i, [vp, vp, i, i, i, i, vp, i, i, vp]),
    "tv_av1_txfm_last_error": (cstr, []),
    "tv_gpu_av1_txfm": (i, [vp, vp, i, i, i, vp, vp, vp]),
    "tv_av1e_last_error": (cstr, []),
    "tv_av1e_inter": (i, [vp] * 18 + [i, i, i, vp, vp]),
    "tv_av1e_iblocks": (i, [vp] * 16 + [i, i, i, vp, i, vp]),
    "tv_av1e_intra": (i, [vp] * 11 + [i, i, i, vp, i, vp]),
    "tv_av1e_cdef_skip": (i, [vp, vp, i, i, i, vp]),
    "tv_av1e_merge": (i, [vp, vp, i, i, i, vp]),
    "tv_av1e_tb_len": (i, [vp, vp, l, i, i, i, i, vp, vp]),
    "tv_av1e_tb_pack": (i, [vp, vp, vp, l, i, i, i, i, vp, vp]),
    "tv_av1e_lfinfo": (i, [vp, i, i, i, vp, vp, vp, vp, vp]),
    "tv_av1e_unit_sse": (i, [vp, vp, i, i, i, i, i, vp, vp]),
    "tv_av1e_cdef_choose": (i, [vp, vp, vp, vp, i, i, i, vp, vp, vp, vp, vp]),
}
```

### thinvids_amd/models/hevc.py

```python
from __future__ import annotations

import ctypes as C
import threading
from dataclasses import dataclass

import numpy as np

from .._native import Bytes, check, core_lib, ok, ptr

Frame = tuple


def coded_size(width: int, height: int, ctb: int = 32) -> tuple[int, int]:
    return (width + ctb - 1) // ctb * ctb, (height + ctb - 1) // ctb * ctb


def synth_frame(seed: int, t: int, width: int, height: int) -> Frame:
    y = np.empty((height, width), np.uint8)
    u = np.empty((height // 2, width // 2), np.uint8)
    v = np.empty_like(u)
    core_lib().tv_synth_frame(seed & 0xFFFFFFFF, t, width, height, ptr(y), ptr(u), ptr(v))
    return y, u, v


def psnr(a: np.ndarray, b: np.ndarray) -> float:
    mse = np.mean((a.astype(np.float64) - b.astype(np.float64)) ** 2)
    return float("inf") if mse == 0 else 10.0 * np.log10(255.0 ** 2 / mse)


def psnr_yuv(ref: Frame, dec: Frame) -> dict:
    py, pu, pv = (psnr(r, d) for r, d in zip(ref, dec))
    return {"y": py, "u": pu, "v": pv, "yuv": (6 * py + pu + pv) / 8}


FLAG_DEBLOCK = 1
FLAG_SAO = 2
FLAG_WPP = 4
FLAG_NO_RQT = 8
FLAG_NO_PINTRA = 16
FLAG_HOST_ENTROPY = 32
FLAG_CASCADE = 64
FLAG_NO_RDOQ = 128
FLAG_SUBPEL_SATD = 256
FLAG_SIGN_HIDING = 512


def codec_flags(deblock: bool = True, sao: bool = False, wpp: bool = True, rqt: bool = True, pintra: bool = True,
                cascade: bool = False, rdoq: bool = True, subpel_satd: bool = False, sign_hiding: bool = False) -> int:
    on = {FLAG_DEBLOCK: deblock, FLAG_SAO: sao, FLAG_WPP: wpp, FLAG_NO_RQT: not rqt, FLAG_NO_PINTRA: not pintra,
          FLAG_CASCADE: cascade, FLAG_NO_RDOQ: not rdoq, FLAG_SUBPEL_SATD: subpel_satd, FLAG_SIGN_HIDING: sign_hiding}
    return sum(bit for bit, v in on.items() if v)


IPPP_CASCADE_IDR = -5
IPPP_CASCADE_P = (1, 0, 1, -1, 1, 0, 1, -3)


def ippp_cascade_qps(qp: int, nframes: int) -> list[int]:
    return [max(0, min(51, qp + (IPPP_CASCADE_IDR if i == 0 else IPPP_CASCADE_P[(i - 1) % 8]))) for i in range(nframes)]


class CpuEncoder:

    def __init__(self, width: int, height: int, qp: int = 27, deblock: bool = True,
                 search_range: int = 64, max_merge: int = 5, sao: bool = False, crf: int = 0, wpp: bool = True,
                 bframes: int = 1, rqt: bool = True, pintra: bool = True, cascade: bool = True, rdoq: bool = True,
                 subpel_satd: bool = False, sign_hiding: bool = False):
        if width % 2 or height % 2:
            raise ValueError("width/height must be even")
        self.lib = core_lib()
        self.width, self.height, self.qp = width, height, qp
        self.cw, self.ch = coded_size(width, height)
        self.bframes = int(bframes)
        flags = codec_flags(deblock, sao, wpp, rqt, pintra, cascade, rdoq, subpel_satd, sign_hiding)
        if self.bframes > 1:
            if crf:
                raise ValueError("CRF with B frames is not supported by the golden encoder")
            self.h = self.lib.tv_cpu_encoder_new_b(width, height, qp, flags, search_range, max_merge, self.bframes)
        elif crf:
            self.h = self.lib.tv_cpu_encoder_new_crf(width, height, qp, flags, search_range, max_merge, int(crf))
        else:
            self.h = self.lib.tv_cpu_encoder_new(width, height, qp, flags, search_range, max_merge)
        if not self.h:
            raise ValueError(self.lib.tv_last_error().decode())
        self.out = Bytes()

    def __del__(self):
        if getattr(self, "h", None):
            self.lib.tv_cpu_encoder_free(self.h)
            self.h = None

    def begin_gop(self, nframes: int) -> list[int]:
        disp = (C.c_int * nframes)()
        check(self.lib.tv_cpu_encoder_begin_gop(self.h, nframes, disp))
        return list(disp)

    def encode(self, frame: Frame, idr: bool, poc: int, qp: int | None = None) -> bytes:
        y, u, v = (np.ascontiguousarray(p) for p in frame)
        self.out.clear()
        if qp is None:
            check(self.lib.tv_cpu_encoder_encode(self.h, ptr(y), ptr(u), ptr(v), y.shape[1], u.shape[1],
                                                 int(idr), poc, self.out.h))
        else:
            check(self.lib.tv_cpu_encoder_encode_qp(self.h, ptr(y), ptr(u), ptr(v), y.shape[1], u.shape[1], int(idr),
                                                    poc, int(qp), self.out.h))
        return self.out.tobytes()

    def recon(self) -> Frame:
        y = np.empty((self.ch, self.cw), np.uint8)
        u = np.empty((self.ch // 2, self.cw // 2), np.uint8)
        v = np.empty_like(u)
        self.lib.tv_cpu_encoder_recon(self.h, ptr(y), ptr(u), ptr(v))
        return y, u, v

    def decisions(self) -> dict:
        w8, h8 = self.cw // 8, self.ch // 8
        d = {k: np.empty((h8, w8), np.uint8) for k in ("cu_log2", "intra", "ipm", "cbf")}
        mv = np.empty((h8, w8, 2), np.int16)
        self.lib.tv_cpu_encoder_decisions(self.h, ptr(d["cu_log2"]), ptr(d["intra"]), ptr(d["ipm"]), ptr(mv),
                                          ptr(d["cbf"]))
        d["mv"] = mv
        return d

    def levels(self) -> tuple:
        cy = np.empty((self.ch, self.cw), np.int16)
        cu = np.empty((self.ch // 2, self.cw // 2), np.int16)
        cv = np.empty_like(cu)
        self.lib.tv_cpu_encoder_levels(self.h, ptr(cy), ptr(cu), ptr(cv))
        return cy, cu, cv


def gop_plan(nframes: int, bframes: int) -> dict:
    lib = core_lib()
    arrs = [(C.c_int * max(1, nframes))() for _ in range(5)]
    info = (C.c_int * 2)()
    n = lib.tv_gop_plan(nframes, bframes, *arrs, info)
    keys = ("disp", "type", "ref0", "ref1", "layer")
    out = {k: list(a)[:n] for k, a in zip(keys, arrs)}
    out["dpb_size"], out["num_reorder"] = info[0], info[1]
    return out


def encode_sequence_cpu(frames, qp: int = 27, gop: int = 0, frame_qps=None, bframes: int = 1,
                        **kw) -> tuple[bytes, list]:
    frames = list(frames)
    h, w = frames[0][0].shape
    if bframes > 1:
        enc = CpuEncoder(w, h, qp=qp, bframes=bframes, **kw)
        seg = gop if gop > 0 else len(frames)
        out, recons = bytearray(), [None] * len(frames)
        for s0 in range(0, len(frames), seg):
            n = min(seg, len(frames) - s0)
            for d in enc.begin_gop(n):
                i = s0 + d
                out += enc.encode(frames[i], d == 0, d, None if frame_qps is None else int(frame_qps[i]))
                recons[i] = enc.recon()
        return bytes(out), recons
    enc = CpuEncoder(w, h, qp=qp, **kw)
    out, recons, poc = bytearray(), [], 0
    for i, f in enumerate(frames):
        idr = i == 0 or (gop > 0 and i % gop == 0)
        poc = 0 if idr else poc + 1
        out += enc.encode(f, idr, poc, None if frame_qps is None else int(frame_qps[i]))
        recons.append(enc.recon())
    return bytes(out), recons


def display_offsets(annexb: bytes) -> np.ndarray:
    lib = core_lib()
    buf = np.frombuffer(annexb, np.uint8)
    cap = max(1, annexb.count(b"\x00\x00\x01"))
    out = np.zeros(cap, np.int32)
    n = lib.tv_hevc_display_offsets(ptr(buf), len(buf), ptr(out), cap)
    if n < 0:
        raise ValueError(lib.tv_last_error().decode())
    return out[:n]


@dataclass
class DecodedStream:
    width: int
    height: int
    coded_w: int
    coded_h: int
    frames: list
    coded_frames: list


def probe_annexb(annexb: bytes) -> dict:
    lib = core_lib()
    buf = np.frombuffer(annexb, np.uint8)
    w, h, n, k = (C.c_int() for _ in range(4))
    check(lib.tv_hevc_probe(ptr(buf), len(annexb), C.byref(w), C.byref(h), C.byref(n), C.byref(k)))
    return {"width": w.value, "height": h.value, "frames": n.value, "idrs": k.value}


def decode(annexb: bytes, coded: bool = True, first: int = 0, count: int = -1) -> DecodedStream:
    lib = core_lib()
    h = lib.tv_decoder_new()
    try:
        buf = np.frombuffer(annexb, np.uint8)
        check(lib.tv_decoder_decode_range(h, ptr(buf), len(annexb), int(first), int(count)))
        w, hh, cw, ch, n = (C.c_int() for _ in range(5))
        lib.tv_decoder_info(h, C.byref(w), C.byref(hh), C.byref(cw), C.byref(ch), C.byref(n))
        frames, coded_frames = [], []
        for i in range(n.value):
            for crop, sink, (W, H) in ((1, frames, (w.value, hh.value)),
                                       (0, coded_frames, (cw.value, ch.value))):
                if crop == 0 and not coded:
                    continue
                y = np.empty((H, W), np.uint8)
                u = np.empty((H // 2, W // 2), np.uint8)
                v = np.empty_like(u)
                check(lib.tv_decoder_frame(h, i, crop, ptr(y), ptr(u), ptr(v)))
                sink.append((y, u, v))
        return DecodedStream(w.value, hh.value, cw.value, ch.value, frames, coded_frames)
    finally:
        lib.tv_decoder_free(h)


def write_frame(width: int, height: int, qp: int, idr: bool, poc: int, dec: dict,
                coef: tuple, deblock: bool = True, max_merge: int = 5, sign_hiding: bool = False) -> bytes:
    lib = core_lib()
    out = Bytes()
    cy, cu, cv = (np.ascontiguousarray(c, dtype=np.int16) for c in coef)
    check(lib.tv_write_frame(width, height, qp, codec_flags(deblock, wpp=False, sign_hiding=sign_hiding), max_merge, int(idr), poc,
                             ptr(np.ascontiguousarray(dec["cu_log2"])), ptr(np.ascontiguousarray(dec["intra"])),
                             ptr(np.ascontiguousarray(dec["ipm"])),
                             ptr(np.ascontiguousarray(dec["mv"], dtype=np.int16)),
                             ptr(np.ascontiguousarray(dec["cbf"])), ptr(cy), ptr(cu),
                             ptr(cv), out.h))
    return out.tobytes()


def reconstruct_reference(width: int, height: int, qp: int, src: Frame, ref: Frame | None,
                          dec: dict, deblock: bool = True, sign_hiding: bool = False):
    lib = core_lib()
    cw, ch = coded_size(width, height)
    cbf = np.zeros((ch // 8, cw // 8), np.uint8)
    cy = np.zeros((ch, cw), np.int16)
    cu = np.zeros((ch // 2, cw // 2), np.int16)
    cv = np.zeros_like(cu)
    ry = np.zeros((ch, cw), np.uint8)
    ru = np.zeros((ch // 2, cw // 2), np.uint8)
    rv = np.zeros_like(ru)
    s = [np.ascontiguousarray(p) for p in src]
    r = [np.ascontiguousarray(p) for p in ref] if ref is not None else None
    null = C.cast(None, C.POINTER(C.c_uint8))
    check(lib.tv_reconstruct_frame(
        width, height, qp, codec_flags(deblock, wpp=False, sign_hiding=sign_hiding), ptr(s[0]), ptr(s[1]), ptr(s[2]),
        ptr(r[0]) if r else null, ptr(r[1]) if r else null, ptr(r[2]) if r else null,
        ptr(np.ascontiguousarray(dec["cu_log2"])), ptr(np.ascontiguousarray(dec["intra"])),
        ptr(np.ascontiguousarray(dec["ipm"])), ptr(np.ascontiguousarray(dec["mv"], dtype=np.int16)),
        ptr(cbf), ptr(cy), ptr(cu), ptr(cv), ptr(ry), ptr(ru), ptr(rv)))
    return cbf, (cy, cu, cv), (ry, ru, rv)


def mux_mp4(annexb: bytes, width: int, height: int, fps_num: int = 30, fps_den: int = 1) -> bytes:
    lib = core_lib()
    out = Bytes()
    buf = np.frombuffer(annexb, np.uint8).copy()
    check(lib.tv_mux_mp4(ptr(buf), len(annexb), width, height, fps_num, fps_den, out.h))
    return out.tobytes()


def mux_mp4_file(segments, width: int, height: int, fps_num: int, fps_den: int, path: str) -> int:
    lib = core_lib()
    segs = [s for s in segments if len(s)]
    keep = [np.frombuffer(s, np.uint8) for s in segs]
    ptrs = (C.c_void_p * len(keep))(*[k.ctypes.data for k in keep])
    sizes = (C.c_size_t * len(keep))(*[len(k) for k in keep])
    out = C.c_ulonglong()
    check(lib.tv_mux_mp4_file(ptrs, sizes, len(keep), width, height, fps_num, fps_den, path.encode(), C.byref(out)))
    return int(out.value)


class Mp4StreamWriter:

    def __init__(self, path: str, width: int, height: int, fps_num: int, fps_den: int, max_samples: int):
        lib = core_lib()
        self.lib, self.path = lib, path
        self.h = lib.tv_mp4s_open(path.encode(), width, height, fps_num, fps_den, max(1, int(max_samples)))
        if not self.h:
            raise RuntimeError(lib.tv_mp4s_last_error().decode())
        self.payload = 0
        self.lock = threading.Lock()

    def append(self, segment) -> None:
        buf = np.frombuffer(segment, np.uint8)
        if not len(buf):
            return
        with self.lock:
            if not self.h:
                raise RuntimeError("stream writer closed")
            ok(self.lib.tv_mp4s_append(self.h, ptr(buf), len(buf)), self.lib, "tv_mp4s_last_error")
        self.payload += len(buf)

    def close(self) -> int:
        with self.lock:
            h, self.h = self.h, None
            if not h:
                raise RuntimeError("stream writer closed")
            out = C.c_ulonglong()
            ok(self.lib.tv_mp4s_close(h, C.byref(out)), self.lib, "tv_mp4s_last_error")
        return int(out.value)

    def abort(self) -> None:
        with self.lock:
            if self.h:
                self.lib.tv_mp4s_abort(self.h)
                self.h = None

    def __del__(self):
        self.abort()


def demux_mp4(data: bytes) -> dict:
    lib = core_lib()
    out = Bytes()
    buf = np.frombuffer(data, np.uint8).copy()
    w, h, n, ts, d = (C.c_int() for _ in range(5))
    check(lib.tv_demux_mp4(ptr(buf), len(data), C.byref(w), C.byref(h), C.byref(n), C.byref(ts),
                           C.byref(d), out.h))
    return {"annexb": out.tobytes(), "width": w.value, "height": h.value, "frames": n.value,
            "timescale": ts.value, "sample_delta": d.value,
            "fps": ts.value / d.value if d.value else 0.0}
```

### thinvids_amd/ops/stage.py

```python
from __future__ import annotations

import ctypes as C
import threading
from dataclasses import dataclass, field

import numpy as np

from .._native import gpu_lib, ok, stream
from ..models.hevc import coded_size


_lib = gpu_lib


def _ok(rc: int, which: str = "stage") -> None:
    ok(rc, gpu_lib(), f"tv_{which}_last_error")


@dataclass
class DevFrames:
    buf: object
    n: int
    w: int
    h: int
    planes: list
    bits: int = 8
    keep: list = field(default_factory=list)

    def ptr(self, c: int) -> int:
        return self.buf.data_ptr() + self.planes[c][0] * self.buf.element_size()

    def select(self, f0: int, n: int) -> "DevFrames":
        pl = [(off + f0 * fs, pw, ph, st, fs) for off, pw, ph, st, fs in self.planes]
        return DevFrames(self.buf, n, self.w, self.h, pl, self.bits, self.keep)


def flat_layout(w: int, h: int) -> list:
    ysz, csz = w * h, (w // 2) * (h // 2)
    fsz = ysz + 2 * csz
    return [(0, w, h, w, fsz), (ysz, w // 2, h // 2, w // 2, fsz), (ysz + csz, w // 2, h // 2, w // 2, fsz)]


_STATS_LOCK = threading.Lock()


class _Pinned:

    _tls = threading.local()

    @classmethod
    def get(cls, nbytes: int):
        import torch

        b = getattr(cls._tls, "buf", None)
        if b is None or b.numel() < nbytes:
            b = torch.empty(max(nbytes, 1 << 20), dtype=torch.uint8).pin_memory()
            cls._tls.buf = b
        return b


def from_flat(t, w: int, h: int, n: int | None = None, bits: int = 8) -> DevFrames:
    n = n if n is not None else t.shape[0]
    return DevFrames(t, n, w, h, flat_layout(w, h), bits)


def thumbs8(ptr: int, bits: int, w: int, h: int, stride: int, fs: int, n: int, out) -> None:
    _ok(_lib().tv_thumbs8_batch(ptr, bits, w, h, stride, fs, n, out.data_ptr(), stream(out.device)))


def upload_frames(frames, device) -> DevFrames:
    import torch

    n = len(frames)
    h, w = frames[0][0].shape
    dt = frames[0][0].dtype
    bits = 10 if dt == np.uint16 else 8
    lay = flat_layout(w, h)
    fsz = lay[0][4]
    esz = 2 if bits == 10 else 1
    pin = _Pinned.get(n * fsz * esz)
    host = pin[: n * fsz * esz].numpy().view(np.int16 if bits == 10 else np.uint8).reshape(n, fsz)
    ysz, csz = w * h, (w // 2) * (h // 2)
    for k, (y, u, v) in enumerate(frames):
        host[k, :ysz] = y.reshape(-1)
        host[k, ysz:ysz + csz] = u.reshape(-1)
        host[k, ysz + csz:] = v.reshape(-1)
    tdt = torch.int16 if bits == 10 else torch.uint8
    dev = torch.empty((n, fsz), dtype=tdt, device=device)
    dev.copy_(pin[: n * fsz * esz].view(tdt).view(n, fsz), non_blocking=True)
    torch.cuda.current_stream(device).synchronize()
    return DevFrames(dev, n, w, h, lay, bits)


def synth_frames(seed: int, w: int, h: int, starts, device) -> DevFrames:
    import torch

    n = len(starts)
    cw, ch = coded_size(w, h)
    ysz, csz = cw * ch, (cw // 2) * (ch // 2)
    buf = torch.empty(n * (ysz + 2 * csz), dtype=torch.uint8, device=device)
    ts = (C.c_int * n)(*[int(t) for t in starts])
    _ok(_lib().tv_synth_batch(buf.data_ptr(), w, h, n, ts, seed & 0xFFFFFFFF, stream(device)))
    planes = [(0, w, h, cw, ysz), (n * ysz, w // 2, h // 2, cw // 2, csz),
              (n * ysz + n * csz, w // 2, h // 2, cw // 2, csz)]
    return DevFrames(buf, n, w, h, planes, 8)


def tone_map(src: DevFrames, src_peak: float = 1000.0, dst_peak: float = 100.0) -> DevFrames:
    import torch

    if src.bits != 10:
        return src
    n, w, h = src.n, src.w, src.h
    dev = src.buf.device
    (yo, _, _, ys, yfs), (uo, _, _, us, ufs), (vo, _, _, vs, vfs) = src.planes
    flat = src.buf.reshape(-1)

    def plane(off, pw, ph, stride, fs):
        return torch.as_strided(flat, (n, ph, pw), (fs, stride, 1), off).to(torch.int32)

    y16 = (plane(yo, w, h, ys, yfs) << 6).to(torch.int16).contiguous()
    u = plane(uo, w // 2, h // 2, us, ufs) << 6
    v = plane(vo, w // 2, h // 2, vs, vfs) << 6
    uv16 = torch.stack([u, v], -1).reshape(n, h // 2, w).to(torch.int16).contiguous()
    fsz = w * h * 3 // 2
    out = torch.empty((n, fsz), dtype=torch.uint8, device=dev)
    _ok(_lib().tv_tonemap_pq_batch(y16.data_ptr(), uv16.data_ptr(), w, h, n, out.data_ptr(), src_peak, dst_peak,
                                   stream(dev)), "ops")
    res = DevFrames(out, n, w, h, flat_layout(w, h), 8)
    res.keep = [y16, uv16]
    return res


def staging_planes(w: int, h: int, coded: tuple | None = None) -> tuple[int, list]:
    cw, ch = coded or coded_size(w, h)
    ysz, csz = cw * ch, (cw // 2) * (ch // 2)
    return ysz + 2 * csz, [(0, w, h, cw, cw, ch), (ysz, w // 2, h // 2, cw // 2, cw // 2, ch // 2),
                           (ysz + csz, w // 2, h // 2, cw // 2, cw // 2, ch // 2)]


def to_staging(src: DevFrames, out_w: int, out_h: int, dst, frame0: int = 0, coded: tuple | None = None) -> None:
    import torch

    from ..models.abr import _tables, resize2d_plan

    src = tone_map(src)
    lib = _lib()
    dev = dst.device
    st = stream(dev)
    fsz, planes = staging_planes(out_w, out_h, coded)
    base = dst.data_ptr() + frame0 * fsz
    for c, (doff, dw, dh, dstride, pw, ph) in enumerate(planes):
        _, sw, sh, sstride, sfs = src.planes[c]
        sp = src.ptr(c)
        if (sw, sh) == (dw, dh):
            _ok(lib.tv_pad_batch(sp, sw, sh, sstride, sfs, base + doff, pw, ph, dstride, fsz, src.n, st))
            continue
        ix, wx, tx = _tables(sw, dw, 3, dev.index)
        iy, wy, ty = _tables(sh, dh, 3, dev.index)
        th, wp, smem = resize2d_plan(sw, sh, dw, dh, pw, ph)
        tmp = torch.empty(1 if th else src.n * sh * dw, dtype=torch.int16, device=dev)
        _ok(lib.tv_resize_batch(sp, sw, sh, sstride, sfs, base + doff, dw, dh, dstride, fsz, pw, ph, src.n,
                                ix.data_ptr(), wx.data_ptr(), tx, iy.data_ptr(), wy.data_ptr(), ty, tmp.data_ptr(),
                                th, wp, smem, st), "ops")


INGEST_CHUNK = 32 << 20


def read_y4m_device(src, start: int, n: int, device, threads: int | None = None, stats: dict | None = None) -> DevFrames:
    import os

    import torch

    info = src.info
    n = max(0, min(n, src.nframes - start))
    nbytes = n * info.frame_bytes
    lib = _lib()
    if threads is None:
        threads = max(1, min(12, len(os.sched_getaffinity(0))))
    ring = _Pinned.get(2 * threads * INGEST_CHUNK)
    esz = 2 if info.bits > 8 else 1
    buf = torch.empty(nbytes // esz, dtype=torch.int16 if esz == 2 else torch.uint8, device=device)
    tm = (C.c_double * 2)()
    if lib.tv_ingest_h2d(src.path.encode(), info.header_len + start * info.frame_bytes, nbytes, buf.data_ptr(),
                         ring.data_ptr(), ring.numel(), threads, stream(device), tm) != 0:
        raise RuntimeError(f"{src.path}: ingest of frames {start}..{start + n} failed: "
                           f"{lib.tv_ingest_last_error().decode()}")
    w, h = info.width, info.height
    hdr = (info.frame_bytes - w * h * 3 // 2 * esz) // esz
    fs = info.frame_bytes // esz
    ysz, csz = w * h, (w // 2) * (h // 2)
    planes = [(hdr, w, h, w, fs), (hdr + ysz, w // 2, h // 2, w // 2, fs), (hdr + ysz + csz, w // 2, h // 2, w // 2, fs)]
    if stats is not None:
        with _STATS_LOCK:
            stats["read_bytes"] = stats.get("read_bytes", 0) + nbytes
            stats["ingest_s"] = stats.get("ingest_s", 0.0) + tm[1]
            stats["read_thread_s"] = stats.get("read_thread_s", 0.0) + tm[0]
            stats["read_threads"] = threads
    return DevFrames(buf, n, w, h, planes, 8 if esz == 1 else 10)


def write_synth_y4m(path: str, w: int, h: int, n: int, seed: int = 1, device=0, chunk: int = 64) -> int:
    import os

    import torch

    dev = torch.device("cuda", device) if isinstance(device, int) else device
    fsz = w * h * 3 // 2
    tmp = path + ".tmp"
    with open(tmp, "wb") as f:
        f.write(f"YUV4MPEG2 W{w} H{h} F30:1 Ip A1:1 C420jpeg\n".encode())
        for t0 in range(0, n, chunk):
            k = min(chunk, n - t0)
            src = synth_frames(seed, w, h, list(range(t0, t0 + k)), dev)
            flat = src.buf.reshape(-1)
            out = torch.empty((k, 6 + fsz), dtype=torch.uint8, device=dev)
            out[:, :6] = torch.tensor(list(b"FRAME\n"), dtype=torch.uint8, device=dev)
            o = 6
            for off, pw, ph, stride, fs in src.planes:
                out[:, o:o + pw * ph] = torch.as_strided(flat, (k, ph, pw), (fs, stride, 1), off).reshape(k, -1)
                o += pw * ph
            f.write(memoryview(out.cpu().numpy()).cast("B"))
    os.replace(tmp, path)
    return os.path.getsize(path)
```

Baseline: 11910.

## Restructure SAO kernel to process strips of four CTUs per workgroup

The SAO decide/filter kernel now handles a horizontal strip of four CTUs per workgroup, one wave per CTU, instead of one CTU per 256-thread workgroup. Edge-offset statistics come from a row-walking loop that reuses the neighbour rows already loaded and uses packed 16-bit arithmetic with a masked boundary variant. The reduction is reworked around permlane and DPP operations. The intent is to cut redundant shared-memory staging and the per-CTU workgroup overhead, and to let more workgroups fit per CU. The change also adds CPU and GPU test entry points for SAO, at the cost of a considerably more complex kernel and indexing.

```diff
diff --git a/csrc/core/capi.cpp b/csrc/core/capi.cpp
--- a/csrc/core/capi.cpp
+++ b/csrc/core/capi.cpp
@@ -142,6 +142,31 @@
 }
 
 int tv_satd8x8(const int* d, int stride) { return satd8x8(d, stride); }
+
+int tv_sao_picture_cpu(int W, int H, int qp, const uint8_t* sy, const uint8_t* su, const uint8_t* sv,
+                       const uint8_t* dy, const uint8_t* du, const uint8_t* dv, uint32_t* params, uint8_t* oy,
+                       uint8_t* ou, uint8_t* ov) {
+  if (W <= 0 || H <= 0 || W % kCtb || H % kCtb || qp < 0 || qp > 51) {
+    g_err = "tv_sao_picture_cpu: bad geometry or QP";
+    return -1;
+  }
+  return guard([&] {
+    Picture src, deb;
+    src.alloc(W, H);
+    deb.alloc(W, H);
+    const uint8_t* s[3] = {sy, su, sv};
+    const uint8_t* d[3] = {dy, du, dv};
+    uint8_t* o[3] = {oy, ou, ov};
+    for (int c = 0; c < 3; ++c) {
+      const size_t n = (size_t)src.pw(c) * src.ph(c);
+      std::memcpy(src.plane(c), s[c], n);
+      std::memcpy(deb.plane(c), d[c], n);
+    }
+    sao_decide_picture(src, deb, qp, params);
+    sao_picture(deb, params);
+    for (int c = 0; c < 3; ++c) std::memcpy(o[c], deb.plane(c), (size_t)deb.pw(c) * deb.ph(c));
+  });
+}
 
 void* tv_cpu_encoder_new(int width, int height, int qp, int deblock, int range, int max_merge) {
   SeqConfig cfg;
diff --git a/csrc/gpu/k_frame.hip b/csrc/gpu/k_frame.hip
--- a/csrc/gpu/k_frame.hip
+++ b/csrc/gpu/k_frame.hip
@@ -500,17 +500,18 @@
   dim3 grid((g.W + 16 + 31) / 32, (g.H + 16 + 31) / 32, B);
   k_phase_planes<<<grid, 256, 0, s>>>(ref, phase, g);
 }
-constexpr int kSaoT = 34;
-constexpr int kSaoTc = 18;
-constexpr int kSaoP = kSaoT + 2, kSaoPc = kSaoTc + 2;
-constexpr int kSaoTile = kSaoT * kSaoP + 2 * kSaoTc * kSaoPc;
-constexpr int kSaoStage = (kSaoTile + 255) / 256;
-__device__ __forceinline__ int sao_tix(int c, int row, int col) {
-  return c == 0 ? row * kSaoP + col + 1 : kSaoT * kSaoP + (c - 1) * kSaoTc * kSaoPc + row * kSaoPc + col + 1;
-}
+constexpr int kSaoStrip = 4;
+constexpr int kSaoRows = 34, kSaoRowsC = 18;
+constexpr int kSaoPd = 16 * kSaoStrip + 2, kSaoPdC = 8 * kSaoStrip + 2;
+constexpr int kSaoLumaDw = kSaoRows * kSaoPd, kSaoChromaDw = kSaoRowsC * kSaoPdC;
+constexpr int kSaoTileDw = kSaoLumaDw + 2 * kSaoChromaDw;
+constexpr int kSaoSrcDw = 8 * kSaoStrip + 2, kSaoSrcDwC = 4 * kSaoStrip + 2;
+static_assert(kSaoSrcDw <= 64 && kSaoSrcDwC <= 32, "a tile row is staged by one wave (chroma: one half per plane)");
+static_assert(8 * (kSaoTileDw * 4 + 64) <= 160 * 1024, "8 workgroups per CU");
 typedef short sao_s2 __attribute__((ext_vector_type(2)));
 __device__ __forceinline__ sao_s2 sao_pair(uint32_t w) { return __builtin_bit_cast(sao_s2, w); }
 typedef unsigned short sao_u2 __attribute__((ext_vector_type(2)));
+__device__ __forceinline__ sao_u2 sao_upair(sao_s2 w) { return __builtin_bit_cast(sao_u2, w); }
 __device__ __forceinline__ sao_s2 sao_sign2(sao_s2 d) {
   const sao_s2 z = {0, 0};
   const sao_u2 f = {15, 15};
@@ -527,322 +528,360 @@
   asm("v_pk_min_i16 %0, %1, %2" : "=v"(r) : "v"(__builtin_bit_cast(uint32_t, a)), "v"(__builtin_bit_cast(uint32_t, b)));
   return sao_pair(r);
 }
-
-__device__ __forceinline__ void sao_tile_pos(int i, int& c, int& j) {
-  c = i < kSaoT * kSaoT ? 0 : (i < kSaoT * kSaoT + kSaoTc * kSaoTc ? 1 : 2);
-  j = c == 0 ? i : i - kSaoT * kSaoT - (c - 1) * kSaoTc * kSaoTc;
-}
-
-__global__ void __launch_bounds__(256) k_sao_decide(FrameSet src, FrameSet deb, FrameSet out, uint32_t* sao, Geo g,
-                                                    const int8_t* qp, const RcTables* rc,
-                                                    unsigned long long* sse) {
-  const int tid = threadIdx.x, lane = tid & 63;
-  int ctu, b;
-  xcd_ctb(ctu, b);
-  const long long lam16 = rc->sao_lam16[qp[b]];
-  const int cx = ctu % g.wc, cy = ctu / g.wc;
-  __shared__ SaoStats st[3];
-  __shared__ __align__(16) int16_t tile[kSaoTile];
-  __shared__ int bpos[3];
-  __shared__ int bh[3][32][16];
-  for (int i = tid; i < 3 * (int)(sizeof(SaoStats) / 4); i += 256) reinterpret_cast<int*>(st)[i] = 0;
-  if (kSaoBandOffsets)
-    for (int i = tid; i < 3 * 32 * 16; i += 256) (&bh[0][0][0])[i] = 0;
-  {
-    uint32_t* tile32 = reinterpret_cast<uint32_t*>(tile);
-    uint32_t v[3];
-    int at[3], dw[3], nd[3];
-    bool act[3], in[3];
-#pragma unroll
-    for (int k = 0; k < 3; ++k) {
-      int c, row, d;
-      if (k < 2) {
-        const int i = tid + 256 * k;
-        c = 0;
-        row = i / 10;
-        d = i - 10 * row;
-        act[k] = i < 34 * 10;
-      } else {
-        const int pl = tid >= 108 ? 1 : 0, j = tid - 108 * pl;
-        c = 1 + pl;
-        row = j / 6;
-        d = j - 6 * row;
-        act[k] = tid < 2 * 108;
-      }
-      const int n = c ? 16 : 32, w = c ? g.W / 2 : g.W, h = c ? g.H / 2 : g.H;
-      const int x = cx * n - 4 + 4 * d, y = cy * n - 1 + row;
-      in[k] = act[k] && x >= 0 && x < w && y >= 0 && y < h;
-      v[k] = in[k] ? *reinterpret_cast<const uint32_t*>(deb.plane(c, b, g) + (long)y * w + x) : 0u;
-      at[k] = (sao_tix(c, row, -1) >> 1) + 2 * d - 1;
-      dw[k] = d;
-      nd[k] = c ? 6 : 10;
-    }
-#pragma unroll
-    for (int k = 0; k < 3; ++k) {
-      if (!act[k]) continue;
-      const uint32_t lo = in[k] ? __builtin_amdgcn_perm(0u, v[k], 0x0c010c00u) : 0xFFFFFFFFu;
-      const uint32_t hi = in[k] ? __builtin_amdgcn_perm(0u, v[k], 0x0c030c02u) : 0xFFFFFFFFu;
-      if (dw[k] >= 1) tile32[at[k]] = lo;
-      if (dw[k] < nd[k] - 1) tile32[at[k] + 1] = hi;
-    }
-  }
-  const int wave = __builtin_amdgcn_readfirstlane(tid >> 6);
-  const int c = wave < 2 ? 0 : wave - 1;
-  const int n = c ? 16 : 32, w = c ? g.W / 2 : g.W;
-  const int nsh = c ? 4 : 5;
-  const int iters = c ? 4 : 8;
-  const uint8_t* S = src.plane(c, b, g) + (long)(cy * n) * w + cx * n;
-  static_assert(!kSaoBandOffsets, "the packed statistics carry no band histogram");
-  const bool interior = cx > 0 && cy > 0 && cx < g.wc - 1 && cy < g.hc - 1;
-  const int piters = c ? 2 : 4;
-  int sv[8] = {};
-  uint32_t sp[4] = {};
-  if (interior) {
-#pragma unroll
-    for (int k = 0; k < 4; ++k) {
-      const int pidx = lane + 64 * k;
-      const int ly = (c == 0 ? wave * 16 : 0) + (pidx >> (nsh - 1)), lx = 2 * (pidx & ((n >> 1) - 1));
-      sp[k] = k < piters ? *reinterpret_cast<const uint16_t*>(S + ly * w + lx) : 0u;
-    }
-  } else {
-#pragma unroll
-    for (int k = 0; k < 8; ++k) {
-      const int i = (c == 0 ? wave * 512 : 0) + lane + 64 * k;
-      sv[k] = k < iters ? S[(i >> nsh) * w + (i & (n - 1))] : 0;
-    }
-  }
-  __syncthreads();
-  int eo[4][4];
-  if (interior) {
-    const uint32_t* tile32 = reinterpret_cast<const uint32_t*>(tile);
-    sao_s2 acc[4][4];
-#pragma unroll
-    for (int d = 0; d < 4; ++d)
-#pragma unroll
-      for (int q = 0; q < 4; ++q) acc[d][q] = sao_s2{0, 0};
-    const sao_s2 zero = {0, 0}, one = {1, 1}, mone = {-1, -1}, sixteen = {16, 16};
-#pragma unroll
-    for (int k = 0; k < 4; ++k) {
-      if (k >= piters) break;
-      const int pidx = lane + 64 * k;
-      const int ly = (c == 0 ? wave * 16 : 0) + (pidx >> (nsh - 1)), lx = 2 * (pidx & ((n >> 1) - 1));
-      uint32_t Pv[3], Cv[3], Nv[3];
-#pragma unroll
-      for (int r = 0; r < 3; ++r) {
-        const int i0 = sao_tix(c, ly + r, lx + 1) >> 1;
-        Pv[r] = tile32[i0 - 1];
-        Cv[r] = tile32[i0];
-        Nv[r] = tile32[i0 + 1];
-      }
-      sao_s2 L[3], R[3], Cc[3];
-#pragma unroll
-      for (int r = 0; r < 3; ++r) {
-        L[r] = sao_pair(__builtin_amdgcn_alignbyte(Cv[r], Pv[r], 2));
-        R[r] = sao_pair(__builtin_amdgcn_alignbyte(Nv[r], Cv[r], 2));
-        Cc[r] = sao_pair(Cv[r]);
-      }
-      const sao_s2 v = Cc[1];
-      const uint32_t o = sp[k];
-      const sao_s2 orig = {(short)(o & 255), (short)(o >> 8)};
-      const sao_s2 w = (orig - v) * sixteen + one;
-      const sao_s2 A[4] = {L[1], Cc[0], L[0], R[0]}, Bn[4] = {R[1], Cc[2], R[2], L[2]};
-#pragma unroll
-      for (int d = 0; d < 4; ++d) {
-        const sao_s2 e = sao_pkmin(sao_pkmax(v - A[d], mone), one) + sao_pkmin(sao_pkmax(v - Bn[d], mone), one);
-        const sao_s2 pos = sao_pkmax(e, zero), neg = sao_pkmax(zero - e, zero);
-        const sao_s2 is[4] = {neg >> one, neg & one, pos & one, pos >> one};
-#pragma unroll
-        for (int q = 0; q < 4; ++q) acc[d][q] += w * is[q];
-      }
-    }
-#pragma unroll
-    for (int d = 0; d < 4; ++d)
-#pragma unroll
-      for (int q = 0; q < 4; ++q) {
-        const int F = __builtin_amdgcn_sdot2(acc[d][q], one, 0, false), C = F & 15;
-        eo[d][q] = (F - C) * 128 + C;
-      }
-  } else {
-    unsigned long long eo64[4] = {0, 0, 0, 0};
-#pragma unroll
-    for (int k = 0; k < 8; ++k) {
-      if (k >= iters) break;
-      const int i = (c == 0 ? wave * 512 : 0) + lane + 64 * k;
-      const int lx = i & (n - 1), ly = i >> nsh;
-      const int v = tile[sao_tix(c, ly + 1, lx + 1)];
-      const int d16 = (sv[k] - v) * 16 + 1;
-      const unsigned long long p64 = (unsigned long long)(long long)d16;
-#pragma unroll
-      for (int d = 0; d < 4; ++d) {
-        int dx, dy;
-        sao_eo_dir(d, dx, dy);
-        const int a = tile[sao_tix(c, ly + 1 + dy, lx + 1 + dx)], bb = tile[sao_tix(c, ly + 1 - dy, lx + 1 - dx)];
-        const int e = tv_min(tv_max(v - a, -1), 1) + tv_min(tv_max(v - bb, -1), 1);
-        const int f = e + 2 - (e > 0);
-        eo64[d] += (a >= 0 && bb >= 0 && e != 0) ? p64 << (16 * f) : 0ull;
-      }
-      if (kSaoBandOffsets) atomicAdd(&bh[c][v >> 3][lane & 15], (sv[k] - v) * 2048 + 1);
+__device__ __forceinline__ sao_s2 sao_clamp1(sao_s2 d) {
+  return sao_pkmin(sao_pkmax(d, sao_s2{-1, -1}), sao_s2{1, 1});
+}
+
+template <bool MASK, int ROWS, int PD>
+__device__ __forceinline__ void sao_walk(const uint32_t* t, const uint32_t (&sp)[ROWS], sao_u2 (&acc)[4][4]) {
+  sao_s2 L0, C0, R0, L1, C1, R1, L2, C2, R2;
+  auto row = [&](int r, sao_s2& L, sao_s2& C, sao_s2& R) {
+    const uint32_t Pv = t[r * PD - 1], Cv = t[r * PD], Nv = t[r * PD + 1];
+    L = sao_pair(__builtin_amdgcn_alignbyte(Cv, Pv, 2));
+    R = sao_pair(__builtin_amdgcn_alignbyte(Nv, Cv, 2));
+    C = sao_pair(Cv);
+  };
+  row(0, L0, C0, R0);
+  row(1, L1, C1, R1);
+  const sao_s2 zero = {0, 0}, one = {1, 1}, sixteen = {16, 16};
+  const sao_u2 uone = {1, 1};
+  sao_s2 pdn = sao_clamp1(C0 - C1);
+#pragma unroll
+  for (int r = 0; r < ROWS; ++r) {
+    row(r + 2, L2, C2, R2);
+    const sao_s2 v = C1;
+    const sao_s2 orig = sao_pair(__builtin_amdgcn_perm(0u, sp[r], 0x0c010c00u));
+    const sao_u2 w = sao_upair((orig - v) * sixteen + one);
+    const sao_s2 dn = sao_clamp1(v - C2);
+    sao_s2 e[4] = {sao_clamp1(v - L1) + sao_clamp1(v - R1), dn - pdn, sao_clamp1(v - L0) + sao_clamp1(v - R2),
+                   sao_clamp1(v - R0) + sao_clamp1(v - L2)};
+    pdn = dn;
+    if (MASK) {
+      e[0] *= sao_pkmin(sao_pkmin(L1, R1), zero) + one;
+      e[1] *= sao_pkmin(sao_pkmin(C0, C2), zero) + one;
+      e[2] *= sao_pkmin(sao_pkmin(L0, R2), zero) + one;
+      e[3] *= sao_pkmin(sao_pkmin(R0, L2), zero) + one;
     }
 #pragma unroll
     for (int d = 0; d < 4; ++d) {
-      unsigned long long acc = eo64[d];
-#pragma unroll
-      for (int q = 0; q < 4; ++q) {
-        const int fv = (int)(int16_t)(acc & 0xffffu);
-        acc = (acc - (unsigned long long)(long long)fv) >> 16;
-        const int cnt = fv & 15;
-        eo[d][q] = ((fv - cnt) >> 4) * 2048 + cnt;
-      }
-    }
-  }
-  {
-    int t[16];
-#pragma unroll
-    for (int k = 0; k < 16; ++k) t[k] = eo[k >> 2][k & 3];
+      const sao_s2 pos = sao_pkmax(e[d], zero), neg = pos - e[d];
+      const sao_u2 up = sao_upair(pos), un = sao_upair(neg);
+      acc[d][0] += w * (un >> uone);
+      acc[d][1] += w * un;
+      acc[d][2] += w * up;
+      acc[d][3] += w * (up >> uone);
+    }
+    L0 = L1, C0 = C1, R0 = R1;
+    L1 = L2, C1 = C2, R1 = R2;
+  }
+}
+__device__ __forceinline__ void sao_counters(const sao_u2 (&acc)[4][4], int (&t)[16]) {
+  const sao_u2 two = {2, 2};
+#pragma unroll
+  for (int d = 0; d < 4; ++d) {
+    const sao_u2 x[4] = {acc[d][0], acc[d][1] - two * acc[d][0], acc[d][2] - two * acc[d][3], acc[d][3]};
+#pragma unroll
+    for (int q = 0; q < 4; ++q) {
+      const uint32_t xv = __builtin_bit_cast(uint32_t, x[q]);
+      const int cn = __builtin_amdgcn_sdot2(sao_pair(xv & 0x000F000Fu), sao_s2{-127, -127}, 0, false);
+      t[4 * d + q] = __builtin_amdgcn_sdot2(sao_pair(xv), sao_s2{128, 128}, cn, false);
+    }
+  }
+}
+template <bool HALF>
+__device__ __forceinline__ int sao_reduce16(int (&t)[16], int lane) {
+  if (!HALF) {
 #pragma unroll
     for (int j = 0; j < 8; ++j) {
       const auto r = __builtin_amdgcn_permlane32_swap((unsigned)t[j], (unsigned)t[j + 8], false, false);
       t[j] = (int)(r[0] + r[1]);
     }
-#pragma unroll
-    for (int j = 0; j < 4; ++j) {
-      const auto r = __builtin_amdgcn_permlane16_swap((unsigned)t[j], (unsigned)t[j + 4], false, false);
-      t[j] = (int)(r[0] + r[1]);
-    }
-    const int m8 = -((lane >> 3) & 1), m4 = -((lane >> 2) & 1);
-#pragma unroll
-    for (int j = 0; j < 2; ++j) {
-      const int x = (t[j] ^ t[j + 2]) & m8;
-      t[j] = (t[j] ^ x) + dpp::mov<dpp::kRowRor8>(t[j + 2] ^ x);
-    }
+  }
+  constexpr int n16 = HALF ? 8 : 4, n8 = n16 / 2, n4 = n8 / 2;
+#pragma unroll
+  for (int j = 0; j < n16; ++j) {
+    const auto r = __builtin_amdgcn_permlane16_swap((unsigned)t[j], (unsigned)t[j + n16], false, false);
+    t[j] = (int)(r[0] + r[1]);
+  }
+  const int m8 = -((lane >> 3) & 1), m4 = -((lane >> 2) & 1), m2 = -((lane >> 1) & 1);
+#pragma unroll
+  for (int j = 0; j < n8; ++j) {
+    const int x = (t[j] ^ t[j + n8]) & m8;
+    t[j] = (t[j] ^ x) + dpp::mov<dpp::kRowRor8>(t[j + n8] ^ x);
+  }
+#pragma unroll
+  for (int j = 0; j < n4; ++j) {
+    const int x = (t[j] ^ t[j + n4]) & m4;
+    t[j] = (t[j] ^ x) + __shfl_xor(t[j + n4] ^ x, 4, 64);
+  }
+  int tot;
+  if (HALF) {
+    const int x = (t[0] ^ t[1]) & m2;
+    tot = (t[0] ^ x) + dpp::mov<dpp::kQuadXor2>(t[1] ^ x);
+  } else {
+    tot = t[0];
+    tot += dpp::mov<dpp::kQuadXor2>(tot);
+  }
+  tot += dpp::mov<dpp::kQuadXor1>(tot);
+  return tot;
+}
+template <int CTRL>
+__device__ __forceinline__ long long sao_dpp_add64(long long v) {
+  const unsigned lo = (unsigned)dpp::mov<CTRL>((int)v), hi = (unsigned)dpp::mov<CTRL>((int)(v >> 32));
+  return v + (long long)((unsigned long long)hi << 32 | lo);
+}
+__device__ __forceinline__ long long sao_readlane64(long long v, int l) {
+  const unsigned lo = (unsigned)__builtin_amdgcn_readlane((int)v, l), hi = (unsigned)__builtin_amdgcn_readlane((int)(v >> 32), l);
+  return (long long)((unsigned long long)hi << 32 | lo);
+}
+
+template <int S>
+__device__ __forceinline__ uint32_t sao_shifted(const uint32_t (&W)[4], int k) {
+  if constexpr (S == 0) return W[k + 1];
+  if constexpr (S < 0) return __builtin_amdgcn_alignbyte(W[k + 1], W[k], 2);
+  if constexpr (S > 0) return __builtin_amdgcn_alignbyte(W[k + 2], W[k + 1], 2);
+}
+template <int CLS, int PD>
+__device__ __forceinline__ uint32_t sao_eo_dword(const uint32_t* t, int i0, uint32_t p) {
+  constexpr int dx = CLS == 1 ? 0 : (CLS == 3 ? 1 : -1), dy = CLS == 0 ? 0 : -1;
+  const int ra = i0 + dy * PD, rb = i0 - dy * PD;
+  const uint32_t Wa[4] = {t[ra - 1], t[ra], t[ra + 1], t[ra + 2]};
+  const uint32_t Wb[4] = {t[rb - 1], t[rb], t[rb + 1], t[rb + 2]};
+  const uint32_t Cv[2] = {t[i0], t[i0 + 1]};
+  const uint32_t t0 = ((p >> 7) & 15) | ((p >> 11) & 15) << 8 | 8u << 16 | ((p >> 15) & 15) << 24;
+  const uint32_t t1 = (p >> 19) & 15;
+  const sao_s2 two = {2, 2}, eight = {8, 8};
+  const sao_u2 u8s = {8, 8};
+  uint32_t r2[2];
+#pragma unroll
+  for (int k = 0; k < 2; ++k) {
+    const sao_s2 v = sao_pair(Cv[k]);
+    const sao_s2 A = sao_pair(sao_shifted<dx>(Wa, k)), B = sao_pair(sao_shifted<-dx>(Wb, k));
+    const sao_s2 inv = (A | B) >> 15;
+    const sao_s2 e = (sao_sign2(v - A) + sao_sign2(v - B)) & ~inv;
+    const uint32_t sel = __builtin_bit_cast(uint32_t, e + two) | 0x0c000c00u;
+    const sao_s2 off = sao_pair(__builtin_amdgcn_perm(t1, t0, sel));
+    const sao_s2 r = sao_relu2(v + off - eight);
+    r2[k] = __builtin_bit_cast(uint32_t, r | (sao_s2{0, 0} - __builtin_bit_cast(sao_s2, __builtin_bit_cast(sao_u2, r) >> u8s)));
+  }
+  return __builtin_amdgcn_perm(r2[1], r2[0], 0x06040200u);
+}
+template <int PD>
+__device__ __forceinline__ uint32_t sao_filter_dword(const uint32_t* t, int i0, uint32_t p) {
+  static_assert(!kSaoBandOffsets, "the SAO filter has no band-offset path");
+  if (sao_type(p) == 2) {
+    switch (sao_class(p)) {
+      case 0: return sao_eo_dword<0, PD>(t, i0, p);
+      case 1: return sao_eo_dword<1, PD>(t, i0, p);
+      case 2: return sao_eo_dword<2, PD>(t, i0, p);
+      default: return sao_eo_dword<3, PD>(t, i0, p);
+    }
+  }
+  return __builtin_amdgcn_perm(t[i0 + 1], t[i0], 0x06040200u);
+}
+__device__ __forceinline__ unsigned sao_sse_dword(uint32_t sw, uint32_t word, int x0, int dwc) {
+  unsigned e2 = 0;
+  if (x0 + 4 <= dwc) {
+#pragma unroll
+    for (int h = 0; h < 2; ++h) {
+      const uint32_t sel = h ? 0x0c030c02u : 0x0c010c00u;
+      const sao_s2 d = sao_pair(__builtin_amdgcn_perm(0u, sw, sel)) - sao_pair(__builtin_amdgcn_perm(0u, word, sel));
+      const sao_u2 dd = __builtin_bit_cast(sao_u2, d * d);
+      e2 = __builtin_amdgcn_udot2(dd, sao_u2{1, 1}, e2, false);
+    }
+  } else {
+#pragma unroll
+    for (int q = 0; q < 4; ++q) {
+      const int d = (int)((sw >> (8 * q)) & 255) - (int)((word >> (8 * q)) & 255);
+      e2 += x0 + q < dwc ? (unsigned)(d * d) : 0u;
+    }
+  }
+  return e2;
+}
+
+__global__ void __launch_bounds__(64 * kSaoStrip, 8) k_sao_decide(FrameSet src, FrameSet deb, FrameSet out, uint32_t* sao,
+                                                               Geo g, const int8_t* qp, const RcTables* rc,
+                                                               unsigned long long* sse) {
+  static_assert(!kSaoBandOffsets, "the statistics carry no band histogram, the decision no band window or argmin");
+  constexpr int S = kSaoStrip;
+  const int tid = threadIdx.x, lane = tid & 63;
+  const int wave = __builtin_amdgcn_readfirstlane(tid >> 6);
+  int strip, b;
+  xcd_ctb(strip, b);
+  const int spr = (g.wc + S - 1) / S;
+  const int sx = strip % spr, cy = strip / spr, cx = sx * S + wave;
+  const bool active = cx < g.wc;
+  const long long lam16 = rc->sao_lam16[qp[b]];
+  __shared__ __align__(16) uint32_t tile[kSaoTileDw];
+  __shared__ unsigned long long esum[3];
+  if (tid < 3) esum[tid] = 0;
+  const int cw = g.W / 2;
+  const int rgY = lane >> 4, pY = lane & 15;
+  const int cp = lane >> 5, rgC = (lane >> 3) & 3, pC = lane & 7;
+  uint32_t spY[8];
+  {
+    constexpr int nY = (kSaoRows + S - 1) / S, nC = (kSaoRowsC + S - 1) / S;
+    uint32_t vy[nY], vc[nC];
+    bool iy[nY], ic[nC];
+    const int dY = lane, xY = sx * (32 * S) - 4 + 4 * dY;
+    const bool colY = dY < kSaoSrcDw && xY >= 0 && xY < g.W;
+    const uint8_t* PY = deb.plane(0, b, g);
+#pragma unroll
+    for (int i = 0; i < nY; ++i) {
+      const int row = wave + S * i, y = cy * 32 - 1 + row;
+      iy[i] = colY && row < kSaoRows && y >= 0 && y < g.H;
+      vy[i] = iy[i] ? *reinterpret_cast<const uint32_t*>(PY + (long)y * g.W + xY) : 0u;
+    }
+    const int dC = lane & 31, xC = sx * (16 * S) - 4 + 4 * dC;
+    const bool colC = dC < kSaoSrcDwC && xC >= 0 && xC < cw;
+    const uint8_t* PC = deb.plane(1 + cp, b, g);
+#pragma unroll
+    for (int i = 0; i < nC; ++i) {
+      const int row = wave + S * i, y = cy * 16 - 1 + row;
+      ic[i] = colC && row < kSaoRowsC && y >= 0 && y < g.H / 2;
+      vc[i] = ic[i] ? *reinterpret_cast<const uint32_t*>(PC + (long)y * cw + xC) : 0u;
+    }
+    const uint8_t* SY = src.plane(0, b, g) + (long)(cy * 32 + 8 * rgY) * g.W + cx * 32 + 2 * pY;
+#pragma unroll
+    for (int r = 0; r < 8; ++r) spY[r] = active ? *reinterpret_cast<const uint16_t*>(SY + r * g.W) : 0u;
+#pragma unroll
+    for (int i = 0; i < nY; ++i) {
+      const int row = wave + S * i;
+      if (row >= kSaoRows || dY >= kSaoSrcDw) continue;
+      const uint32_t lo = iy[i] ? __builtin_amdgcn_perm(0u, vy[i], 0x0c010c00u) : 0xFFFFFFFFu;
+      const uint32_t hi = iy[i] ? __builtin_amdgcn_perm(0u, vy[i], 0x0c030c02u) : 0xFFFFFFFFu;
+      uint32_t* T = tile + row * kSaoPd + 2 * dY;
+      if (dY >= 1) T[-1] = lo;
+      if (dY < kSaoSrcDw - 1) T[0] = hi;
+    }
+#pragma unroll
+    for (int i = 0; i < nC; ++i) {
+      const int row = wave + S * i;
+      if (row >= kSaoRowsC || dC >= kSaoSrcDwC) continue;
+      const uint32_t lo = ic[i] ? __builtin_amdgcn_perm(0u, vc[i], 0x0c010c00u) : 0xFFFFFFFFu;
+      const uint32_t hi = ic[i] ? __builtin_amdgcn_perm(0u, vc[i], 0x0c030c02u) : 0xFFFFFFFFu;
+      uint32_t* T = tile + kSaoLumaDw + cp * kSaoChromaDw + row * kSaoPdC + 2 * dC;
+      if (dC >= 1) T[-1] = lo;
+      if (dC < kSaoSrcDwC - 1) T[0] = hi;
+    }
+  }
+  __syncthreads();
+  unsigned e2[3] = {0, 0, 0};
+  if (active) {
+    const bool interior = cx > 0 && cy > 0 && cx < g.wc - 1 && cy < g.hc - 1;
+    const uint32_t* tY = tile + wave * 16 + 1;
+    const uint32_t* tC0 = tile + kSaoLumaDw + wave * 8 + 1;
+    int totY, totC;
     {
-      const int x = (t[0] ^ t[1]) & m4;
-      t[0] = (t[0] ^ x) + __shfl_xor(t[1] ^ x, 4, 64);
-    }
-    int tot = t[0];
-    tot += dpp::mov<dpp::kQuadXor1>(tot);
-    tot += dpp::mov<dpp::kQuadXor2>(tot);
-    const int k = lane >> 2;
-    if ((lane & 3) == 0 && (tot & 2047)) {
-      atomicAdd(&st[c].eo_n[k >> 2][(k & 3) + 1], tot & 2047);
-      atomicAdd(&st[c].eo_s[k >> 2][(k & 3) + 1], (tot - (tot & 2047)) / 2048);
-    }
-  }
-  __shared__ SaoTables tab;
-  __shared__ uint32_t prm[3];
-  __syncthreads();
-  if (kSaoBandOffsets && tid < 96) {
-    const int cc = tid >> 5, band = tid & 31;
-    int tot = 0;
-#pragma unroll
-    for (int k = 0; k < 16; ++k) tot += bh[cc][band][k];
-    st[cc].bo_n[band] = tot & 2047;
-    st[cc].bo_s[band] = (tot - (tot & 2047)) / 2048;
-  }
-  __syncthreads();
-  if (tid < kSaoItems && (kSaoBandOffsets || tid % 48 < 16)) sao_item(st, lam16, tid, tab);
-  __syncthreads();
-  if (kSaoBandOffsets && tid < 96) sao_window(tid, tab);
-  __syncthreads();
-  if (!kSaoBandOffsets) {
-    if (tid < 3) bpos[tid] = 0;
-  } else if (wave < 3) {
-    long long j = lane < 32 ? tab.win_j[wave][lane] : LLONG_MAX;
-    int p = lane < 32 ? lane : 64;
-#pragma unroll
-    for (int o = 32; o >= 1; o >>= 1) {
-      const long long j2 = __shfl_xor(j, o);
-      const int p2 = __shfl_xor(p, o);
-      if (j2 < j || (j2 == j && p2 < p)) {
-        j = j2;
-        p = p2;
-      }
-    }
-    if (lane == 0) bpos[wave] = p;
-  }
-  __syncthreads();
-  if (tid == 0) {
-    sao_finish_pos(tab, lam16, bpos, prm);
-    uint32_t* o = sao + 3 * ((long)b * g.wc * g.hc + ctu);
-    o[0] = prm[0];
-    o[1] = prm[1];
-    o[2] = prm[2];
-  }
-  __syncthreads();
-  static_assert(!kSaoBandOffsets, "the SAO filter has no band-offset path");
-  unsigned e2[3] = {0, 0, 0};
-  const uint32_t* tile32 = reinterpret_cast<const uint32_t*>(tile);
-  for (int i = tid; i < 256 + 128; i += 256) {
-    const int cc = i < 256 ? 0 : (i < 320 ? 1 : 2);
-    const int j = cc == 0 ? i : i - 256 - (cc - 1) * 64;
-    const int nd = cc ? 4 : 8, nn = cc ? 16 : 32, ww = cc ? g.W / 2 : g.W;
-    const int ly = j >> (cc ? 2 : 3), lx0 = 4 * (j & (nd - 1));
-    const uint32_t p = prm[cc];
-    const long at = (long)(cy * nn + ly) * ww + cx * nn + lx0;
-    const int dwc = cc ? g.dw / 2 : g.dw, dhc = cc ? g.dh / 2 : g.dh;
-    const bool want_sse = sse && cy * nn + ly < dhc;
-    const uint32_t sw = want_sse ? *reinterpret_cast<const uint32_t*>(src.plane(cc, b, g) + at) : 0u;
-    uint32_t word = 0;
-    const int i0 = sao_tix(cc, ly + 1, lx0 + 1) >> 1;
-    const uint32_t C0 = tile32[i0], C1 = tile32[i0 + 1];
-    if (sao_type(p) == 2) {
-      int dx, dy;
-      sao_eo_dir(sao_class(p), dx, dy);
-      const int pd = (cc ? kSaoPc : kSaoP) >> 1;
-      const int ra = i0 + dy * pd, rb = i0 - dy * pd;
-      const uint32_t Wa[4] = {tile32[ra - 1], tile32[ra], tile32[ra + 1], tile32[ra + 2]};
-      const uint32_t Wb[4] = {tile32[rb - 1], tile32[rb], tile32[rb + 1], tile32[rb + 2]};
-      auto shifted = [](const uint32_t* W, int k, int s) -> uint32_t {
-        return s == 0 ? W[k + 1] : s < 0 ? __builtin_amdgcn_alignbyte(W[k + 1], W[k], 2)
-                                         : __builtin_amdgcn_alignbyte(W[k + 2], W[k + 1], 2);
-      };
-      const uint32_t t0 = ((p >> 7) & 15) | ((p >> 11) & 15) << 8 | 8u << 16 | ((p >> 15) & 15) << 24;
-      const uint32_t t1 = (p >> 19) & 15;
-      const sao_s2 two = {2, 2}, eight = {8, 8};
-      const sao_u2 u8s = {8, 8};
-      uint32_t r2[2];
-#pragma unroll
-      for (int k = 0; k < 2; ++k) {
-        const sao_s2 v = sao_pair(k ? C1 : C0);
-        const sao_s2 A = sao_pair(shifted(Wa, k, dx)), B = sao_pair(shifted(Wb, k, -dx));
-        const sao_s2 inv = (A | B) >> 15;
-        const sao_s2 e = (sao_sign2(v - A) + sao_sign2(v - B)) & ~inv;
-        const uint32_t sel = __builtin_bit_cast(uint32_t, e + two) | 0x0c000c00u;
-        const sao_s2 off = sao_pair(__builtin_amdgcn_perm(t1, t0, sel));
-        const sao_s2 r = sao_relu2(v + off - eight);
-        r2[k] = __builtin_bit_cast(uint32_t, r | (sao_s2{0, 0} - __builtin_bit_cast(sao_s2, __builtin_bit_cast(sao_u2, r) >> u8s)));
-      }
-      word = __builtin_amdgcn_perm(r2[1], r2[0], 0x06040200u);
-    } else {
-      word = __builtin_amdgcn_perm(C1, C0, 0x06040200u);
-    }
-    *reinterpret_cast<uint32_t*>(out.plane(cc, b, g) + at) = word;
-    if (want_sse) {
-      if (cx * nn + lx0 + 4 <= dwc) {
-#pragma unroll
-        for (int h = 0; h < 2; ++h) {
-          const uint32_t sel = h ? 0x0c030c02u : 0x0c010c00u;
-          const sao_s2 d = sao_pair(__builtin_amdgcn_perm(0u, sw, sel)) - sao_pair(__builtin_amdgcn_perm(0u, word, sel));
-          const sao_u2 dd = __builtin_bit_cast(sao_u2, d * d);
-          e2[cc] = __builtin_amdgcn_udot2(dd, sao_u2{1, 1}, e2[cc], false);
-        }
-      } else {
-#pragma unroll
-        for (int q = 0; q < 4; ++q) {
-          const int d = (int)((sw >> (8 * q)) & 255) - (int)((word >> (8 * q)) & 255);
-          e2[cc] += cx * nn + lx0 + q < dwc ? (unsigned)(d * d) : 0u;
+      sao_u2 acc[4][4];
+      int t[16];
+      uint32_t spC[4];
+#pragma unroll
+      for (int d = 0; d < 4; ++d)
+#pragma unroll
+        for (int q = 0; q < 4; ++q) acc[d][q] = sao_u2{0, 0};
+      const uint32_t* tp = tY + 8 * rgY * kSaoPd + pY;
+      if (interior)
+        sao_walk<false, 8, kSaoPd>(tp, spY, acc);
+      else
+        sao_walk<true, 8, kSaoPd>(tp, spY, acc);
+      sao_counters(acc, t);
+      totY = sao_reduce16<false>(t, lane);
+#pragma unroll
+      for (int d = 0; d < 4; ++d)
+#pragma unroll
+        for (int q = 0; q < 4; ++q) acc[d][q] = sao_u2{0, 0};
+      tp = tC0 + cp * kSaoChromaDw + 4 * rgC * kSaoPdC + pC;
+      const uint8_t* SC = src.plane(1 + cp, b, g) + (long)(cy * 16 + 4 * rgC) * cw + cx * 16 + 2 * pC;
+#pragma unroll
+      for (int r = 0; r < 4; ++r) spC[r] = *reinterpret_cast<const uint16_t*>(SC + r * cw);
+      if (interior)
+        sao_walk<false, 4, kSaoPdC>(tp, spC, acc);
+      else
+        sao_walk<true, 4, kSaoPdC>(tp, spC, acc);
+      sao_counters(acc, t);
+      totC = sao_reduce16<true>(t, lane);
+    }
+    uint32_t prm[3];
+    {
+      const bool chroma = lane & 1;
+      const int tot = chroma ? totC : totY, k = chroma ? (lane & 31) >> 1 : lane >> 2;
+      const int n = tot & 2047, s = (tot - n) >> 11;
+      const bool pos = (k & 3) < 2;
+      int o;
+      const long long j = sao_best_offset(n, s, pos ? 0 : -kSaoMaxOff, pos ? kSaoMaxOff : 0, lam16, false, o);
+      const uint32_t ob = (uint32_t)(o + 8) << (7 + 4 * (k & 3));
+      const bool ly = (lane & 3) == 0;
+      long long jy = ly ? j : 0, jc = chroma ? j : 0;
+      int py = ly ? (int)ob : 0, pc = chroma ? (int)ob : 0;
+      jy = sao_dpp_add64<dpp::kQuadXor1>(jy);
+      jy = sao_dpp_add64<dpp::kQuadXor2>(jy);
+      jc = sao_dpp_add64<dpp::kQuadXor1>(jc);
+      jc = sao_dpp_add64<dpp::kQuadXor2>(jc);
+      jy = sao_dpp_add64<dpp::kRowHalfMirror>(jy);
+      jc = sao_dpp_add64<dpp::kRowHalfMirror>(jc);
+      jy = sao_dpp_add64<dpp::kRowMirror>(jy);
+      py += dpp::mov<dpp::kQuadXor1>(py);
+      py += dpp::mov<dpp::kQuadXor2>(py);
+      pc += dpp::mov<dpp::kQuadXor1>(pc);
+      pc += dpp::mov<dpp::kQuadXor2>(pc);
+      py += dpp::mov<dpp::kRowHalfMirror>(py);
+      pc += dpp::mov<dpp::kRowHalfMirror>(pc);
+      py += dpp::mov<dpp::kRowMirror>(py);
+      long long best = lam16 * 1;
+      int cls = -1;
+#pragma unroll
+      for (int c2 = 0; c2 < 4; ++c2) {
+        const long long jj = sao_readlane64(jy, 16 * c2) + lam16 * 4;
+        if (jj < best) {
+          best = jj;
+          cls = c2;
         }
       }
+      prm[0] = cls < 0 ? sao_off_param() : 2u | (uint32_t)cls << 2 | (uint32_t)__builtin_amdgcn_readlane(py, 16 * cls);
+      best = lam16 * 1;
+      cls = -1;
+#pragma unroll
+      for (int c2 = 0; c2 < 4; ++c2) {
+        const long long jj = sao_readlane64(jc, 8 * c2) + sao_readlane64(jc, 32 + 8 * c2) + lam16 * 4;
+        if (jj < best) {
+          best = jj;
+          cls = c2;
+        }
+      }
+      prm[1] = cls < 0 ? sao_off_param() : 2u | (uint32_t)cls << 2 | (uint32_t)__builtin_amdgcn_readlane(pc, 8 * cls);
+      prm[2] = cls < 0 ? sao_off_param() : 2u | (uint32_t)cls << 2 | (uint32_t)__builtin_amdgcn_readlane(pc, 32 + 8 * cls);
+      if (lane < 3) sao[3 * ((long)b * g.wc * g.hc + cy * g.wc + cx) + lane] = lane == 0 ? prm[0] : (lane == 1 ? prm[1] : prm[2]);
+    }
+#pragma unroll
+    for (int k = 0; k < 4; ++k) {
+      const int ly = 8 * ((lane >> 3) & 3) + 4 * (lane >> 5) + k, lx0 = 4 * (lane & 7);
+      const long at = (long)(cy * 32 + ly) * g.W + cx * 32 + lx0;
+      const bool want_sse = sse && cy * 32 + ly < g.dh;
+      const uint32_t sw = want_sse ? *reinterpret_cast<const uint32_t*>(src.plane(0, b, g) + at) : 0u;
+      const uint32_t word = sao_filter_dword<kSaoPd>(tY, (ly + 1) * kSaoPd + (lx0 >> 1), prm[0]);
+      *reinterpret_cast<uint32_t*>(out.plane(0, b, g) + at) = word;
+      if (want_sse) e2[0] += sao_sse_dword(sw, word, cx * 32 + lx0, g.dw);
+    }
+#pragma unroll
+    for (int cc = 1; cc < 3; ++cc) {
+      const int ly = 4 * ((lane >> 2) & 3) + (lane >> 4), lx0 = 4 * (lane & 3);
+      const long at = (long)(cy * 16 + ly) * cw + cx * 16 + lx0;
+      const bool want_sse = sse && cy * 16 + ly < g.dh / 2;
+      const uint32_t sw = want_sse ? *reinterpret_cast<const uint32_t*>(src.plane(cc, b, g) + at) : 0u;
+      const uint32_t word =
+          sao_filter_dword<kSaoPdC>(tC0 + (cc - 1) * kSaoChromaDw, (ly + 1) * kSaoPdC + (lx0 >> 1), prm[cc]);
+      *reinterpret_cast<uint32_t*>(out.plane(cc, b, g) + at) = word;
+      if (want_sse) e2[cc] += sao_sse_dword(sw, word, cx * 16 + lx0, g.dw / 2);
     }
   }
   if (sse) {
-    __shared__ unsigned long long esum[3];
-    if (tid < 3) esum[tid] = 0;
-    __syncthreads();
-#pragma unroll
-    for (int c2 = 0; c2 < 3; ++c2) {
-      const int t = wave_sum((int)e2[c2]);
-      if (lane == 0 && t) atomicAdd(&esum[c2], (unsigned long long)(unsigned)t);
+    if (active) {
+#pragma unroll
+      for (int c2 = 0; c2 < 3; ++c2) {
+        const int t = wave_sum((int)e2[c2]);
+        if (lane == 0 && t) atomicAdd(&esum[c2], (unsigned long long)(unsigned)t);
+      }
     }
     __syncthreads();
     if (tid < 3 && esum[tid]) atomicAdd(sse + b * 3 + tid, esum[tid]);
@@ -851,7 +890,8 @@
 
 void launch_sao(FrameSet src, FrameSet deb, FrameSet out, uint32_t* sao, const int8_t* qp, const RcTables* rc,
                 const Geo& g, int B, hipStream_t s, unsigned long long* sse) {
-  k_sao_decide<<<dim3(g.wc * g.hc, B), 256, 0, s>>>(src, deb, out, sao, g, qp, rc, sse);
+  const int strips = (g.wc + kSaoStrip - 1) / kSaoStrip * g.hc;
+  k_sao_decide<<<dim3(strips, B), 64 * kSaoStrip, 0, s>>>(src, deb, out, sao, g, qp, rc, sse);
 }
 
 void launch_deblock(FrameSet rec, DecisionSet dec, const Geo& g, int B, hipStream_t s) {
diff --git a/csrc/gpu/k_stage.hip b/csrc/gpu/k_stage.hip
--- a/csrc/gpu/k_stage.hip
+++ b/csrc/gpu/k_stage.hip
@@ -92,4 +92,44 @@
   }
   return stage_status();
 }
+
+int tv_sao_batch(const uint8_t* src, const uint8_t* deb, uint8_t* out, uint32_t* sao, unsigned long long* sse, int w,
+                 int h, int B, const int8_t* qp, void* stream) {
+  if (w < 2 || h < 2 || (w & 1) || (h & 1) || B <= 0 || B > tv::gpu::kMaxBatch) {
+    g_stage_err = "tv_sao_batch: bad geometry";
+    return -1;
+  }
+  for (int b = 0; b < B; ++b)
+    if (qp[b] < 0 || qp[b] > 51) {
+      g_stage_err = "tv_sao_batch: bad QP";
+      return -1;
+    }
+  using namespace tv::gpu;
+  hipStream_t st = static_cast<hipStream_t>(stream);
+  const Geo g = make_geo(w, h);
+  auto set = [&](const uint8_t* p) {
+    uint8_t* q = const_cast<uint8_t*>(p);
+    return FrameSet{q, q + B * g.ysz, q + B * g.ysz + B * g.csz};
+  };
+  RcTables t{};
+  for (int q = 0; q < 52; ++q) t.sao_lam16[q] = tv::sao_lambda16(q);
+  RcTables* rc = nullptr;
+  int8_t* dqp = nullptr;
+  bool ok = hipMalloc(&rc, sizeof(RcTables)) == hipSuccess && hipMalloc(&dqp, (size_t)B) == hipSuccess &&
+            hipMemcpyAsync(rc, &t, sizeof(RcTables), hipMemcpyHostToDevice, st) == hipSuccess &&
+            hipMemcpyAsync(dqp, qp, (size_t)B, hipMemcpyHostToDevice, st) == hipSuccess &&
+            hipMemsetAsync(sse, 0, (size_t)B * 3 * sizeof(unsigned long long), st) == hipSuccess;
+  if (ok) {
+    launch_sao(set(src), set(deb), set(out), sao, dqp, rc, g, B, st, sse);
+    ok = hipStreamSynchronize(st) == hipSuccess;
+  }
+  const int rcode = stage_status();
+  (void)hipFree(rc);
+  (void)hipFree(dqp);
+  if (rcode == 0 && !ok) {
+    g_stage_err = "tv_sao_batch: device error";
+    return -1;
+  }
+  return rcode;
 }
+}
diff --git a/thinvids_amd/_abi.py b/thinvids_amd/_abi.py
--- a/thinvids_amd/_abi.py
+++ b/thinvids_amd/_abi.py
@@ -26,6 +26,7 @@
     "tv_synth_frame": (None, [u32, i, i, i, u8p, u8p, u8p]),
     "tv_synth_frame_tiled": (None, [u32, i, i, i, i, i, u8p, u8p, u8p]),
     "tv_satd8x8": (i, [i32p, i]),
+    "tv_sao_picture_cpu": (i, [i, i, i] + [u8p] * 6 + [u32p] + [u8p] * 3),
     "tv_cpu_encoder_new": (vp, [i] * 6),
     "tv_cpu_encoder_new_b": (vp, [i] * 7),
     "tv_cpu_encoder_new_crf": (vp, [i] * 7),
@@ -128,6 +129,7 @@
     "tv_thumbs8_batch": (i, [vp, i, i, i, i, l, i, vp, vp]),
     "tv_pad_batch": (i, [vp, i, i, i, l, vp, i, i, i, l, i, vp]),
     "tv_synth_batch": (i, [vp, i, i, i, i32p, u32, vp]),
+    "tv_sao_batch": (i, [vp, vp, vp, vp, vp, i, i, i, i8p, vp]),
     "tv_ops_last_error": (cstr, []),
     "tv_resize_plane": (i, [vp, i, i, i, vp, i, i, i, vp, vp, i, vp, vp, i, vp, vp]),
     "tv_resize_batch": (i, [vp, i, i, i, l, vp, i, i, i, l, i, i, i, vp, vp, i, vp, vp, i, vp, i, i, i, vp]),
diff --git a/thinvids_amd/models/hevc.py b/thinvids_amd/models/hevc.py
--- a/thinvids_amd/models/hevc.py
+++ b/thinvids_amd/models/hevc.py
@@ -21,6 +21,17 @@
     v = np.empty_like(u)
     core_lib().tv_synth_frame(seed & 0xFFFFFFFF, t, width, height, ptr(y), ptr(u), ptr(v))
     return y, u, v
+
+
+def sao_picture_cpu(src: Frame, deb: Frame, qp: int) -> tuple[np.ndarray, Frame]:
+    h, w = deb[0].shape
+    src = [np.ascontiguousarray(p, np.uint8) for p in src]
+    deb = [np.ascontiguousarray(p, np.uint8) for p in deb]
+    params = np.empty((h // 32, w // 32, 3), np.uint32)
+    out = [np.empty_like(p) for p in deb]
+    check(core_lib().tv_sao_picture_cpu(w, h, qp, *[ptr(p) for p in src], *[ptr(p) for p in deb], ptr(params),
+                                        *[ptr(p) for p in out]))
+    return params, tuple(out)
 
 
 def psnr(a: np.ndarray, b: np.ndarray) -> float:
diff --git a/thinvids_amd/ops/stage.py b/thinvids_amd/ops/stage.py
--- a/thinvids_amd/ops/stage.py
+++ b/thinvids_amd/ops/stage.py
@@ -104,6 +104,35 @@
     planes = [(0, w, h, cw, ysz), (n * ysz, w // 2, h // 2, cw // 2, csz),
               (n * ysz + n * csz, w // 2, h // 2, cw // 2, csz)]
     return DevFrames(buf, n, w, h, planes, 8)
+
+
+def sao_pictures(src, deb, w: int, h: int, qps, device):
+    import torch
+
+    B = len(deb)
+    cw, ch = coded_size(w, h)
+
+    def batched(pics):
+        flat = np.concatenate([np.ascontiguousarray(p[c], np.uint8).reshape(-1) for c in range(3) for p in pics])
+        assert flat.size == B * cw * ch * 3 // 2, "pictures must have the coded size"
+        return torch.from_numpy(flat).to(device)
+
+    ds, dd = batched(src), batched(deb)
+    out = torch.empty_like(dd)
+    nctb = (cw // 32) * (ch // 32)
+    prm = torch.empty(B * nctb * 3, dtype=torch.int32, device=device)
+    sse = torch.empty(B * 3, dtype=torch.int64, device=device)
+    q = (C.c_int8 * B)(*[int(x) for x in qps])
+    torch.cuda.current_stream(device).synchronize()
+    _ok(_lib().tv_sao_batch(ds.data_ptr(), dd.data_ptr(), out.data_ptr(), prm.data_ptr(), sse.data_ptr(), w, h, B, q,
+                            stream(device)))
+    o = out.cpu().numpy()
+    ysz, csz = cw * ch, cw * ch // 4
+    pics = [(o[b * ysz:(b + 1) * ysz].reshape(ch, cw),
+             o[B * ysz + b * csz:B * ysz + (b + 1) * csz].reshape(ch // 2, cw // 2),
+             o[B * (ysz + csz) + b * csz:B * (ysz + csz) + (b + 1) * csz].reshape(ch // 2, cw // 2)) for b in range(B)]
+    return (prm.cpu().numpy().view(np.uint32).reshape(B, ch // 32, cw // 32, 3), pics,
+            sse.cpu().numpy().view(np.uint64).reshape(B, 3))
 
 
 def tone_map(src: DevFrames, src_peak: float = 1000.0, dst_peak: float = 100.0) -> DevFrames:
```

Result: faster. 12930, median of 6 (+8.5%).
